# rasmusbarr/nudge

Measured on AMD Instinct MI355X. Metric: simulation steps/s (contacts solved/s alongside), 1M-box drop scene, higher is better.
Workload: dtype f32

## Files before the change

include/nudge_hip.h:

```cpp
#ifndef NUDGE_HIP_H
#define NUDGE_HIP_H

#include <stdint.h>

#ifdef __cplusplus
extern "C" {
#endif

enum {
	NH_OK = 0,
	NH_ERR_INVALID = 1,
	NH_ERR_NO_DEVICE = 2,
	NH_ERR_ARENA = 3,
	NH_ERR_CONTACT_CAPACITY = 4,
	NH_ERR_CACHE_CAPACITY = 5,
	NH_ERR_ACTIVE_CAPACITY = 6,
	NH_ERR_PAIR_CAPACITY = 7,
	NH_ERR_HIP = 8,
	NH_ERR_SCHEDULER_CAPACITY = 9,
	NH_ERR_STALE_HINT = 11,
	NH_ERR_STALE_SETUP = 10
};

enum {
// ... 50 lines not shown
typedef struct nh_ActiveBodies { uint32_t* indices; uint32_t capacity; uint32_t count; } nh_ActiveBodies;

typedef struct nh_ContactImpulseData nh_ContactImpulseData;
typedef struct nh_ContactConstraintData nh_ContactConstraintData;
typedef struct nh_context nh_context;

typedef struct nh_Counts {
	uint32_t colliders;
	uint32_t pairs;
	uint32_t contacts;
	uint32_t sleeping_pairs;
	uint32_t active_bodies;
	uint32_t cache;
	uint32_t culled;
	uint32_t large_colliders;
	uint32_t general_contacts;
	uint32_t levels;
	uint32_t error;
	uint32_t has_other_bodies;
	uint32_t unleveled;
	uint32_t raw_pairs;
	uint32_t broadphase_rebuilds;
	uint32_t sort_reuses;
	uint32_t broadphase_inserts;
	uint32_t still_steps;
	uint32_t still_replays;
	uint32_t still_diff[4];
	uint32_t blk_blocks, blk_bodies, blk_ghosts;
	uint32_t asleep_steps;
	uint32_t ahead_steps;
	uint32_t fused_steps;
	uint32_t pair_steps;
	uint32_t pair_diag[4];
} nh_Counts;

int nh_create(nh_context** out, int device, void* stream, uint32_t flags);
void nh_destroy(nh_context* ctx);
int nh_set_flags(nh_context* ctx, uint32_t flags);
int nh_synchronize(nh_context* ctx);
int nh_read_counts(nh_context* ctx, nh_Counts* out);
enum { NH_VIEW_CONTACTS = 1u , NH_VIEW_CACHE = 2u, NH_VIEW_ACTIVE = 4u , NH_VIEW_ALL = 7u };
int nh_export_views(nh_context* ctx, uint32_t what);
int nh_set_cache_count(nh_context* ctx, uint32_t count);
int nh_bodies_changed(nh_context* ctx);
int nh_set_tag_bits(nh_context* ctx, uint32_t bits);
int nh_set_pair_capacity(nh_context* ctx, uint32_t pairs);
int nh_set_option(nh_context* ctx, const char* name, int value);
const char* nh_error_string(int code);
int nh_last_hip_error(nh_context* ctx);

int nh_collide(nh_context* ctx, nh_ActiveBodies* active_bodies, nh_ContactData* contacts,
               const nh_BodyData* bodies, const nh_ColliderData* colliders,
               const nh_BodyConnections* body_connections, nh_Arena temporary);

int nh_append_contacts(nh_context* ctx, nh_ContactData* contacts, const nh_BodyData* bodies, uint32_t extra, uint32_t* positions, nh_Arena temporary);

int nh_apply_gravity_damping(nh_context* ctx, const nh_ActiveBodies* active_bodies, const nh_BodyData* bodies,
                             float time_step, const float gravity[3], float damping_rate);

int nh_read_cached_impulses(nh_context* ctx, const nh_ContactCache* contact_cache, const nh_ContactData* contacts,
                            nh_Arena* memory, nh_ContactImpulseData** out);

int nh_write_cached_impulses(nh_context* ctx, nh_ContactCache* contact_cache, const nh_ContactData* contacts,
                             nh_ContactImpulseData* contact_impulses);

int nh_setup_contact_constraints(nh_context* ctx, const nh_ActiveBodies* active_bodies, const nh_ContactData* contacts,
// ... 162 lines not shown
```

nudge_amd/csrc/nh_append.hip:

```cpp
#include "nh_internal.h"

__device__ __forceinline__ bool app_less(uint64_t ta, uint32_t fa, uint64_t tb, uint32_t fb) { return ta < tb || (ta == tb && fa < fb); }

__global__ __launch_bounds__(256) void k_app_rank(const nh_DevState* __restrict__ st, uint32_t extra, const uint64_t* __restrict__ tags, const uint32_t* __restrict__ features,
                                                  uint32_t* __restrict__ rank, uint64_t* __restrict__ skey, uint32_t* __restrict__ sfeat, uint32_t capacity) {
	const uint32_t K = st->contacts;
	if ((uint64_t)K + extra > capacity) return;
	for (uint32_t j = blockIdx.x * blockDim.x + threadIdx.x; j < extra; j += gridDim.x * blockDim.x) {
		const uint64_t t = tags[K + j]; const uint32_t f = features[K + j];
		uint32_t r = 0;
		for (uint32_t i = 0; i < extra; ++i) {
			const uint64_t ti = tags[K + i]; const uint32_t fi = features[K + i];
			r += (app_less(ti, fi, t, f) || (ti == t && fi == f && i < j)) ? 1u : 0u;
		}
		rank[j] = r; skey[r] = t; sfeat[r] = f;
	}
}

__global__ __launch_bounds__(256) void k_app_positions(const nh_DevState* __restrict__ st, uint32_t extra, const uint64_t* __restrict__ tags, const uint32_t* __restrict__ features,
                                                       const uint32_t* __restrict__ rank, const uint64_t* __restrict__ skey, const uint32_t* __restrict__ sfeat, uint32_t* __restrict__ pos, uint32_t capacity) {
	const uint32_t K = st->contacts;
	if ((uint64_t)K + extra > capacity) return;
	for (uint32_t i = blockIdx.x * blockDim.x + threadIdx.x; i < K + extra; i += gridDim.x * blockDim.x) {
		const uint64_t t = tags[i]; const uint32_t f = features[i];
// ... 26 lines not shown
	if ((uint64_t)st->contacts + extra > capacity) return;
	const uint32_t n = st->contacts + extra;
	for (uint32_t i = blockIdx.x * blockDim.x + threadIdx.x; i < n; i += gridDim.x * blockDim.x) {
		const uint32_t p = pos[i];
		reinterpret_cast<float4*>(data + p)[0] = t_data[2 * (size_t)i]; reinterpret_cast<float4*>(data + p)[1] = t_data[2 * (size_t)i + 1];
		bodies[p] = t_bodies[i]; tags[p] = t_tags[i]; features[p] = t_features[i];
	}
}

__global__ __launch_bounds__(256) void k_app_recount(nh_DevState* __restrict__ st, uint32_t extra, const nh_BodyPair* __restrict__ bodies, const uint64_t* __restrict__ tags,
                                                     uint32_t* __restrict__ deg, uint32_t nbodies, uint32_t capacity) {
	if ((uint64_t)st->contacts + extra > capacity) return;
	unsigned long long* __restrict__ pair_counter = reinterpret_cast<unsigned long long*>(deg + 2u * NH_DEG_STRIDE(nbodies));
	uint32_t* __restrict__ first_contact = deg + 4u * NH_DEG_STRIDE(nbodies);
	const uint32_t n = st->contacts + extra;
	for (uint32_t i = blockIdx.x * blockDim.x + threadIdx.x; i < n; i += gridDim.x * blockDim.x) {
		const nh_BodyPair p = bodies[i];
		if (i > 0 && tags[i - 1] == tags[i] && bodies[i - 1].a == p.a && bodies[i - 1].b == p.b) continue;
		const uint64_t t = tags[i];
		uint32_t len = 1;
		while (i + len < n && tags[i + len] == t && bodies[i + len].a == p.a && bodies[i + len].b == p.b) ++len;
		if (p.a) { atomicAdd(&pair_counter[p.a], (unsigned long long)len | ((unsigned long long)(p.b ? 0x10001u : 1u) << 32)); first_contact[p.a] = i | 0x80000000u; }
		if (p.b) { atomicAdd(&pair_counter[p.b], (unsigned long long)len | ((unsigned long long)(p.a ? 0x10001u : 1u) << 32)); first_contact[p.b] = i; }
	}
}

__global__ void k_app_count(nh_DevState* st, uint32_t extra, uint32_t capacity) {
	if (st->contacts + extra > capacity) st->error = NH_ERR_CONTACT_CAPACITY; else st->contacts += extra;
}

extern "C" int nh_append_contacts(nh_context* ctx, nh_ContactData* contacts, const nh_BodyData* bodies, uint32_t extra, uint32_t* positions, nh_Arena temporary) {
	if (!ctx || !contacts || !bodies) return NH_ERR_INVALID;
	if (!extra) return NH_OK;
	if (extra > 65536u || extra > contacts->capacity) return NH_ERR_INVALID;
	if (ctx->setup_seq == ctx->collide_seq || !ctx->deg) return NH_ERR_STALE_SETUP;
	{ int rc = nh_flush_pending(ctx); if (rc) return rc; }
	{ int rc = nh_still_sync_outputs(ctx); if (rc) return rc; }
	ctx->still.appended = true; ctx->still.ok_next = false;
	nh_DevState* st = ctx->d_state;
	const uint32_t cap = contacts->capacity, B = bodies->count;
	int err = NH_OK;
	uint32_t* rank = nh_arena_array<uint32_t>(&temporary, extra, &err);
	uint64_t* skey = nh_arena_array<uint64_t>(&temporary, extra, &err);
	uint32_t* sfeat = nh_arena_array<uint32_t>(&temporary, extra, &err);
	uint32_t* pos = positions ? positions : nh_arena_array<uint32_t>(&temporary, cap, &err);
	float4* t_data = nh_arena_array<float4>(&temporary, 2 * (size_t)cap, &err);
	nh_BodyPair* t_bodies = nh_arena_array<nh_BodyPair>(&temporary, cap, &err);
	uint64_t* t_tags = nh_arena_array<uint64_t>(&temporary, cap, &err);
	uint32_t* t_features = nh_arena_array<uint32_t>(&temporary, cap, &err);
	if (err) return err;
	if ((ctx->flags & NH_FLAG_SYNC_COUNTS) && (uint64_t)contacts->count + extra > cap) return NH_ERR_CONTACT_CAPACITY;
	NH_LAUNCH(ctx, "append_rank", k_app_rank, nh_grid_for(extra, 256, 1024), 256, st, extra, contacts->tags, contacts->features, rank, skey, sfeat, cap);
	NH_LAUNCH(ctx, "append_positions", k_app_positions, nh_grid_for(cap, 256, 2048), 256, st, extra, contacts->tags, contacts->features, rank, skey, sfeat, pos, cap);
	NH_LAUNCH(ctx, "append_copy", k_app_copy, nh_grid_for(cap, 256, 2048), 256, st, extra, contacts->data, contacts->bodies, contacts->tags, contacts->features, t_data, t_bodies, t_tags, t_features, cap);
	NH_LAUNCH(ctx, "append_scatter", k_app_scatter, nh_grid_for(cap, 256, 2048), 256, st, extra, pos, t_data, t_bodies, t_tags, t_features, contacts->data, contacts->bodies, contacts->tags, contacts->features, cap);
	NH_HIP_CHECK(ctx, hipMemsetAsync(ctx->deg, 0, sizeof(uint32_t) * NH_DEG_WORDS(B), ctx->stream));
	NH_LAUNCH(ctx, "append_recount", k_app_recount, nh_grid_for(cap, 256, 2048), 256, st, extra, contacts->bodies, contacts->tags, ctx->deg, B, cap);
	NH_LAUNCH(ctx, "append_count", k_app_count, 1, 1, st, extra, cap);
	if (ctx->flags & NH_FLAG_SYNC_COUNTS) {
		nh_Counts c;
		int rc = nh_read_counts(ctx, &c);
		if (rc) return rc;
		if (c.error) return (int)c.error;
		contacts->count = c.contacts;
	}
	return NH_OK;
// ... 2 lines not shown
```

nudge_amd/csrc/nh_cache.hip:

```cpp
#include "nh_internal.h"

__global__ __launch_bounds__(256) void k_cache_lookup(const nh_DevState* __restrict__ st, const uint64_t* __restrict__ tags, const uint32_t* __restrict__ features,
                                                      const uint64_t* __restrict__ ctags, const uint32_t* __restrict__ cfeatures, const nh_CachedContactImpulse* __restrict__ cdata,
                                                      nh_CachedContactImpulse* __restrict__ out, const nh_BodyPair* __restrict__ bodies, const uint8_t* __restrict__ body_class) {
	uint32_t n = st->contacts, m = st->cache;
	for (uint32_t i = blockIdx.x * blockDim.x + threadIdx.x; i < n; i += gridDim.x * blockDim.x) {
		if (body_class) {
			const nh_BodyPair p = bodies[i];
			const uint32_t ca = p.a ? body_class[p.a] : 0u, cb = p.b ? body_class[p.b] : 0u;
			if (ca != NH_CLS_GENERAL && cb != NH_CLS_GENERAL && ca != NH_CLS_STATICN && cb != NH_CLS_STATICN) continue;
		}
		uint64_t t = tags[i]; uint32_t f = features[i];
		uint32_t lo = 0, hi = m;
		if (i < m && ctags[i] == t && cfeatures[i] == f) { lo = i; hi = i; }
		while (lo < hi) { uint32_t mid = (lo + hi) >> 1; if (tag_less(ctags[mid], cfeatures[mid], t, f)) lo = mid + 1; else hi = mid; }
		nh_CachedContactImpulse r = { { 0.0f, 0.0f, 0.0f }, 0.0f };
		if (lo < m && ctags[lo] == t && cfeatures[lo] == f) r = cdata[lo];
		out[i] = r;
	}
}

__global__ __launch_bounds__(256) void k_cache_lookup_listed(const nh_DevState* __restrict__ st, const uint32_t* __restrict__ list, const uint64_t* __restrict__ tags, const uint32_t* __restrict__ features,
                                                             const uint64_t* __restrict__ ctags, const uint32_t* __restrict__ cfeatures, const nh_CachedContactImpulse* __restrict__ cdata,
                                                             nh_CachedContactImpulse* __restrict__ out) {
// ... 125 lines not shown
	}
}

__global__ __launch_bounds__(256) void k_sleep_undo(uint64_t* __restrict__ sc_undo, uint32_t* __restrict__ sc_count, uint32_t n, uint32_t confirmed_seq) {
	for (uint32_t r = blockIdx.x * blockDim.x + threadIdx.x; r < n; r += gridDim.x * blockDim.x) {
		const uint64_t u = sc_undo[r];
		if (u == 0ull) continue;
		if ((uint32_t)(u >> 32) > confirmed_seq) sc_count[r] = (uint32_t)u;
		sc_undo[r] = 0ull;
	}
}

static nh_ContactImpulseData* new_impulse_data(nh_context* ctx) {
	if (ctx->impulse_ring.empty()) { ctx->impulse_ring.resize(64, nullptr); ctx->constraint_ring.resize(64, nullptr); }
	uint32_t k = ctx->ring_pos % 64;
	if (!ctx->impulse_ring[k]) ctx->impulse_ring[k] = new nh_ContactImpulseData();
	return ctx->impulse_ring[k];
}

void nh_run_cull(nh_context* ctx, nh_ContactImpulseData* d, uint32_t sleeping_on_host) {
	if (!d->cull_pending) return;
	d->cull_pending = false;
	if (sleeping_on_host == 0) return;
	nh_DevState* st = ctx->d_state;
	const uint32_t ccap = d->cache_capacity;
	NH_LAUNCH(ctx, "cull_flags", k_cull_flags, nh_grid_for(ccap, 256, 4096), 256, st, d->ctags, d->sleeping_pairs, d->cull_flags);
	nh_scan_u32(ctx, d->cull_flags, d->cull_flags, &st->cache, 1, d->cull_tmp, &st->culled, &st->sleeping);
	NH_LAUNCH(ctx, "cull_write", k_cull_write, nh_grid_for(ccap, 256, 4096), 256, st, d->cull_flags, d->cull_flags, d->ctags, d->cfeatures, d->cdata,
	          d->culled_tags, d->culled_features, d->culled_data);
}

extern "C" int nh_read_cached_impulses(nh_context* ctx, const nh_ContactCache* cache, const nh_ContactData* contacts, nh_Arena* memory, nh_ContactImpulseData** out) {
	if (!ctx || !cache || !contacts || !memory || !out) return NH_ERR_INVALID;
	{
		const nh_StillStep& ss = ctx->still;
		const bool in_sequence = ss.active && !ss.resolved && !ctx->pending && cache->tags == ss.cache_tags && cache->features == ss.cache_features && cache->data == ss.cache_data &&
		                         cache->capacity == ss.cache_capacity && contacts->data == ss.lay_contacts.data && contacts->tags == ss.lay_contacts.tags;
		int rc = nh_flush_pending(ctx, true, in_sequence); if (rc) return rc;
	}
	const uint32_t kcap = contacts->capacity, ccap = cache->capacity;
	int err = NH_OK;
	ctx->ring_pos++;
	nh_ContactImpulseData* d = new_impulse_data(ctx);
	d->data = nh_arena_array<nh_CachedContactImpulse>(memory, kcap, &err);
	d->culled_tags = nh_arena_array<uint64_t>(memory, ccap, &err);
	d->culled_features = nh_arena_array<uint32_t>(memory, ccap, &err);
	d->culled_data = nh_arena_array<nh_CachedContactImpulse>(memory, ccap, &err);
	d->capacity = kcap; d->culled_capacity = ccap;
	d->cull_flags = nh_arena_array<uint32_t>(memory, ccap + 1, &err);
	d->cull_tmp = nh_arena_array<uint32_t>(memory, 2 * NH_SORT_GRID + 64, &err);
	if (err) return err;
	d->lookup_pending = true; d->ctx = ctx; d->consumed = false;
	d->tags = contacts->tags; d->features = contacts->features;
	d->ctags = cache->tags; d->cfeatures = cache->features; d->cdata = cache->data;
	d->cull_pending = contacts->sleeping_pairs != nullptr;
	d->sleeping_pairs = contacts->sleeping_pairs;
	d->cache_capacity = ccap;
	if (d->cull_pending && (ctx->flags & NH_FLAG_SYNC_COUNTS)) {
		nh_run_cull(ctx, d, ctx->h_state->sleeping);
	}
	*out = d;
	return NH_OK;
}

void nh_materialize_lookup(nh_context* ctx, nh_ContactImpulseData* d, const nh_BodyPair* bodies, const uint8_t* body_class, const uint32_t* general_list, uint32_t general) {
	if (!d->lookup_pending) return;
	d->lookup_pending = false;
	if (general_list && general != 0u && (uint64_t)general * 16u < d->capacity && !ctx->no_listed_lookup) {
		NH_LAUNCH(ctx, "cache_lookup_listed", k_cache_lookup_listed, nh_grid_for(general, 256, 4096), 256, ctx->d_state, general_list, d->tags, d->features, d->ctags, d->cfeatures, d->cdata, d->data);
		return;
	}
	NH_LAUNCH(ctx, "cache_lookup", k_cache_lookup, nh_grid_for(d->capacity, 256, 16384), 256, ctx->d_state, d->tags, d->features, d->ctags, d->cfeatures, d->cdata, d->data, bodies, body_class);
}

extern "C" const nh_CachedContactImpulse* nh_contact_impulses_device(const nh_ContactImpulseData* d) {
	if (!d) return nullptr;
	nh_ContactImpulseData* m = const_cast<nh_ContactImpulseData*>(d);
	if (m->ctx) {
		if (m->ctx->pending) nh_flush_pending(m->ctx);
		else if (!m->consumed) nh_materialize_lookup(m->ctx, m);
		nh_StillStep& ss = m->ctx->still;
		if (ss.active && ss.resolved && m->consumed && m->cdata == ss.cache_data) {
			if (nh_still_sync_outputs(m->ctx, NH_VIEW_CACHE) == NH_OK)
				hipMemcpyAsync(m->data, ss.cache.data, sizeof(nh_CachedContactImpulse) * (size_t)(m->capacity < ss.cache.capacity ? m->capacity : ss.cache.capacity), hipMemcpyDeviceToDevice, m->ctx->stream);
		}
	}
	return d->data;
}

extern "C" int nh_write_cached_impulses(nh_context* ctx, nh_ContactCache* cache, const nh_ContactData* contacts, nh_ContactImpulseData* imp) {
	if (!ctx || !cache || !contacts || !imp) return NH_ERR_INVALID;
	{ int rc = nh_flush_pending(ctx); if (rc) return rc; }
	{
		nh_StillStep& ss = ctx->still;
		if (ss.active && ss.resolved && cache->data == ss.cache_data && imp->ctx == ctx && imp->consumed) return NH_OK;
		ss.cache_ok = imp->consumed && !imp->cull_pending && !(ctx->flags & NH_FLAG_SYNC_COUNTS) && ((ctx->h_state->sleeping == 0u && ctx->h_state->culled == 0u) || !ss.no_local) &&
		              contacts->data == ss.lay_contacts.data && contacts->tags == ss.lay_contacts.tags;
		ss.cache_tags = cache->tags; ss.cache_features = cache->features; ss.cache_data = cache->data; ss.cache_capacity = cache->capacity;
		ss.cache = *cache;
		ss.slots_current = false;
	}
	if (!imp->consumed) nh_materialize_lookup(ctx, imp);
	if (imp->cull_pending) {
		nh_Counts c;
		int rc = nh_read_counts(ctx, &c);
		if (rc) return rc;
		nh_run_cull(ctx, imp, c.sleeping_pairs);
	}
	nh_DevState* st = ctx->d_state;
	NH_LAUNCH(ctx, "write_cache", k_write_cache, nh_grid_for((uint64_t)contacts->capacity + cache->capacity, 256, 4096), 256, st,
	          contacts->tags, contacts->features, imp->data, imp->culled_tags, imp->culled_features, imp->culled_data,
	          cache->tags, cache->features, cache->data, cache->capacity);
	if (ctx->still.ok_next && ctx->still.cache_ok && !ctx->still.disabled && (ctx->flags & NH_FLAG_FUSED_STEP) && ctx->sort_seeded) {
		NH_LAUNCH(ctx, "cache_to_slots", k_cache_to_slots, nh_grid_for(contacts->capacity, 256, 4096), 256, st, ctx->dense_slot, imp->data, contacts->features, ctx->rec,
		          ctx->sc_imp, ctx->sc_feat, ctx->sc_count);
		if (ctx->h_state->sleeping)
			NH_LAUNCH(ctx, "culled_to_slots", k_culled_to_slots, nh_grid_for(imp->culled_capacity, 256, 2048), 256, st, imp->culled_tags, imp->culled_features, imp->culled_data, ctx->sort_sorted_keys,
			          ctx->sort_sorted_idx, ctx->rec, ctx->lay_capacity, ctx->sc_imp, ctx->sc_feat, ctx->sc_count);
		ctx->still.slots_current = true;
	}
	if (ctx->flags & NH_FLAG_SYNC_COUNTS) {
		nh_Counts c;
		int rc = nh_read_counts(ctx, &c);
		if (rc) return rc;
// ... 28 lines not shown
```

nudge_amd/csrc/nh_collide.hip:

```cpp
#include "nh_internal.h"
#include "nh_narrowphase.h"
#include <type_traits>
#include "nh_solver.h"
#include <stdlib.h>

#define NH_ESC_MAX 4096u
#define NH_REINSERT_COMBOS(ncolliders) ((uint64_t)(ncolliders) * 16u)
#define NH_MOVED_MAX 16384u
__device__ __forceinline__ float nh_kept_margin(float cell_inv) { return cell_inv > 0.0f ? 0.03125f / cell_inv : 0.05f; }

template<bool STILL>
__global__ __launch_bounds__(1024) void k_xform(nh_DevState* __restrict__ st,
                                               const nh_Transform* __restrict__ body_xf,
                                               const nh_Transform* __restrict__ box_xf, const nh_BoxCollider* __restrict__ box_data, const uint32_t* __restrict__ box_tags, uint32_t nbox,
                                               const nh_Transform* __restrict__ sph_xf, const nh_SphereCollider* __restrict__ sph_data, const uint32_t* __restrict__ sph_tags, uint32_t nsph,
                                               nh_xform* __restrict__ xf, float4* __restrict__ aabb_min, float4* __restrict__ aabb_max, uint32_t* __restrict__ ctag,
                                               uint4* __restrict__ zero16, uint32_t zero16_count, float4* fat_box, uint32_t direct,
                                               uint8_t* __restrict__ gen, uint32_t* __restrict__ esc_mark, uint32_t* __restrict__ esc_list, uint32_t* __restrict__ moved_list, uint32_t seq,
                                               const uint8_t* __restrict__ idle = nullptr, uint32_t nbodies = 0u, uint32_t parity = 0u, uint8_t* __restrict__ awake_out = nullptr,
                                               uint32_t skip_asleep = 0u) {
	__shared__ uint32_t hist[STILL ? 1 : 1024];
	__shared__ uint32_t red[12];
	__shared__ uint32_t s_asleep;
	if (!STILL) hist[threadIdx.x] = 0;
// ... 1237 lines not shown
					for (int index = 0; index < 16; ++index) {
						if (((bb.mask >> index) & 1u) && k < count) {
							nh_contact_out o;
							nh_bb_contact(bb, index, bb.fx[index], bb.fy[index], bb.fz[index], bb.penetration[index], bb.tags[index], o);
							float4* dp = reinterpret_cast<float4*>(raw_data + base + k);
							dp[0] = make_float4(o.px, o.py, o.pz, o.penetration); dp[1] = make_float4(o.nx, o.ny, o.nz, o.friction);
							raw_feature[base + k] = o.feature;
							++k;
						}
					}
				} else {
					const nh_contact_out o = bb.kind == 1 ? bb.edge : single;
					float4* dp = reinterpret_cast<float4*>(raw_data + base);
					dp[0] = make_float4(o.px, o.py, o.pz, o.penetration); dp[1] = make_float4(o.nx, o.ny, o.nz, o.friction);
					raw_feature[base] = o.feature;
				}
			}
			rec[r].count = (uint32_t)count;
			if (old != (uint32_t)count) {
				cnt_sorted[pos] = (uint32_t)count;
				if (!st->delta_overflow[parity]) {
					const uint32_t k = atomicAdd(&st->delta_count[parity], 1u);
					if (k < NH_DELTA_MAX) delta[parity * NH_DELTA_MAX + k] = make_int2((int)pos, count - (int)old);
					else { st->delta_overflow[parity] = 1u; if (!delta_scan) changed = true; }
				}
			}
		}
		j += stride;
		if (j < n) r = list[j];
	}
	if (__ballot(changed) != 0ull && lane == 0) atomicMax(&st->still_failed_seq, seq);
}

__global__ __launch_bounds__(256) void k_asleep_check(nh_DevState* __restrict__ st, const nh_Transform* __restrict__ body_xf, const uint8_t* __restrict__ idle, uint32_t nbodies,
                                                      const nh_Transform* __restrict__ box_xf, const nh_BoxCollider* __restrict__ box_data, const uint32_t* __restrict__ box_tags, uint32_t nbox,
                                                      const nh_Transform* __restrict__ sph_xf, const nh_SphereCollider* __restrict__ sph_data, const uint32_t* __restrict__ sph_tags, uint32_t nsph,
                                                      const float4* __restrict__ was_min, const float4* __restrict__ was_max, const uint32_t* __restrict__ was_tag) {
	bool differs = false;
	for (uint32_t i = blockIdx.x * blockDim.x + threadIdx.x + 1u; i < nbodies; i += gridDim.x * blockDim.x) differs |= idle[i] != 0xffu;
	const uint32_t n = nbox + nsph;
	for (uint32_t c = blockIdx.x * blockDim.x + threadIdx.x; c < n; c += gridDim.x * blockDim.x) {
		const bool is_box = c < nbox;
		const nh_Transform l = is_box ? box_xf[c] : sph_xf[c - nbox];
		if (l.body >= nbodies) { differs = true; continue; }
		const nh_Transform b = body_xf[l.body];
		const nh_quat bq = { b.rotation[0], b.rotation[1], b.rotation[2], b.rotation[3] };
		const nh_quat lq = { l.rotation[0], l.rotation[1], l.rotation[2], l.rotation[3] };
		const nh_f3 p = nh_rotate(bq, nh_make3(l.position[0], l.position[1], l.position[2])) + nh_make3(b.position[0], b.position[1], b.position[2]);
		const nh_quat q = nh_qmul(bq, lq);
		float sx, sy, sz;
		uint32_t tag;
		if (is_box) {
			const nh_m33 m = nh_matrix(q);
			const nh_BoxCollider bc = box_data[c];
			const nh_f3 c0 = m.c0 * bc.size[0], c1 = m.c1 * bc.size[1], c2 = m.c2 * bc.size[2];
			sx = fabsf(c0.x) + fabsf(c1.x) + fabsf(c2.x);
			sy = fabsf(c0.y) + fabsf(c1.y) + fabsf(c2.y);
			sz = fabsf(c0.z) + fabsf(c1.z) + fabsf(c2.z);
			tag = box_tags[c];
		} else {
			sx = sy = sz = sph_data[c - nbox].radius;
			tag = sph_tags[c - nbox];
		}
		const float4 mn = was_min[c], mx = was_max[c];
		const float mnx = p.x - sx, mny = p.y - sy, mnz = p.z - sz, mxx = p.x + sx, mxy = p.y + sy, mxz = p.z + sz;
		differs |= __float_as_uint(mnx) != __float_as_uint(mn.x) || __float_as_uint(mny) != __float_as_uint(mn.y) || __float_as_uint(mnz) != __float_as_uint(mn.z) ||
// ... 279 lines not shown
	if (t == 0) {
		st->colliders = ncolliders; st->pairs = 0; st->pairs_sph = 0; st->raw_contacts = 0; st->records = 0; st->contacts = 0; st->sleeping = 0;
		st->active = 0; st->culled = 0; st->general_contacts = 0; st->levels = 0; st->error = 0;
		st->has_other = 0; st->has_unstable = 0; st->unleveled = 0; st->has_static8 = 0; st->has_staticN = 0; st->any_sleeping = 0; st->has_pending = 0;
		st->sort_buckets = st->sort_buckets_next;
		st->fat_escaped = 0; st->fat_rebuild = 0; st->esc_count = 0; st->fat_reinsert = 0;
		st->fat_hits_prev = st->fat_hits; st->fat_hits = 0;
		st->keys_changed = 0;
		if (drop_sort_order) st->sort_valid = 0;
		if (drop_kept_pairs) st->fat_valid = 0;
		for (int k = 0; k < 3; ++k) { st->smin[k] = 0xffffffffu; st->smax[k] = 0u; st->gmin[k] = 0xffffffffu; st->gmax[k] = 0u; }
	}
	for (uint32_t k = t; k < 1024u; k += blockDim.x) st->exp_hist[k] = 0;
}

static bool same_bodies(const nh_BodyData& a, const nh_BodyData& b) {
	return a.transforms == b.transforms && a.properties == b.properties && a.momentum == b.momentum && a.idle_counters == b.idle_counters && a.count == b.count;
}
static bool same_colliders(const nh_ColliderData& a, const nh_ColliderData& b) {
	return a.boxes.tags == b.boxes.tags && a.boxes.data == b.boxes.data && a.boxes.transforms == b.boxes.transforms && a.boxes.count == b.boxes.count &&
	       a.spheres.tags == b.spheres.tags && a.spheres.data == b.spheres.data && a.spheres.transforms == b.spheres.transforms && a.spheres.count == b.spheres.count;
}
static bool same_contacts(const nh_ContactData& a, const nh_ContactData& b) {
	return a.data == b.data && a.bodies == b.bodies && a.tags == b.tags && a.features == b.features && a.capacity == b.capacity && a.sleeping_pairs == b.sleeping_pairs;
}

static int collide_impl(nh_context* ctx, nh_ActiveBodies* active_bodies, nh_ContactData* contacts, const nh_BodyData* bodies, const nh_ColliderData* colliders,
                        const nh_BodyConnections* body_connections, nh_Arena temporary, bool want_still);

extern "C" int nh_collide(nh_context* ctx, nh_ActiveBodies* active_bodies, nh_ContactData* contacts,
                          const nh_BodyData* bodies, const nh_ColliderData* colliders,
                          const nh_BodyConnections* body_connections, nh_Arena temporary) {
	if (!ctx || !active_bodies || !contacts || !bodies || !colliders) return NH_ERR_INVALID;
	NH_HIP_CHECK(ctx, hipSetDevice(ctx->device));
	{ int rc = nh_flush_pending(ctx); if (rc) return rc; }
	nh_StillStep& ss = ctx->still;
	ss.active = false; ss.resolved = false; ss.setup_d = nullptr;
	const bool held = ss.hold != 0u;
	if (held) ss.hold--;
	const bool want_still = !held && !ss.disabled && !ctx->first_ghost && ss.ok_next && ss.cache_ok && ss.slots_current && !ss.appended && (ctx->flags & NH_FLAG_FUSED_STEP) && !(ctx->flags & (NH_FLAG_SYNC_COUNTS | NH_FLAG_EXACT_ORDER)) &&
	                        same_bodies(*bodies, ss.lay_bodies) && same_colliders(*colliders, ss.lay_colliders) && same_contacts(*contacts, ss.lay_contacts) &&
	                        active_bodies->indices == ss.lay_active && active_bodies->capacity == ss.lay_active_capacity;
	ss.active_out = active_bodies; ss.contacts_out = contacts; ss.bodies = *bodies; ss.colliders = *colliders;
	ss.has_connections = body_connections != nullptr;
	if (body_connections) ss.connections = *body_connections;
	ss.temporary = temporary;
	return collide_impl(ctx, active_bodies, contacts, bodies, colliders, body_connections, temporary, want_still);
}

int nh_still_collide_again(nh_context* ctx) {
	nh_StillStep& ss = ctx->still;
	const bool after_collide = ctx->after_collide, may_overlap = ctx->gravity_may_overlap;
	ss.active = false; ss.resolved = false; ss.ok_next = false;
	ss.failed++; ss.note_failure();
	ss.replaying = true;
	const int rc = collide_impl(ctx, ss.active_out, ss.contacts_out, &ss.bodies, &ss.colliders, ss.has_connections ? &ss.connections : nullptr, ss.temporary, false);
	ss.replaying = false;
	ctx->after_collide = after_collide; ctx->gravity_may_overlap = may_overlap;
	return rc;
}

int nh_still_view_contacts(nh_context* ctx) {
	const nh_ContactData& c = ctx->still.lay_contacts;
	const uint32_t pair_cap = ctx->lay_capacity;
	NH_LAUNCH(ctx, "gather_contacts", k_gather_contacts, nh_grid_for(pair_cap, 256, 8192), 256, ctx->d_state, ctx->sort_sorted_idx, ctx->rec, ctx->sort_sorted_keys, ctx->start_sorted,
	          ctx->raw_data, ctx->raw_feature, c.data, c.bodies, c.tags, c.features, c.capacity, pair_cap, (const uint32_t*)nullptr, (uint64_t*)nullptr, ctx->deg, ctx->still.bodies.count,
// ... 79 lines not shown
	return ctx->env_no_fat || ctx->bp_direct_left > 0;
}

static int reserve_kept(nh_context* ctx, const CollideCall& c, const CollideScratch& s, bool* fresh) {
	const uint32_t C = c.C, pair_cap = s.pair_cap;
	if (ctx->fat_nbox != c.nbox || ctx->fat_nsph != c.nsph) *fresh = true;
	const uint32_t want_kept = pair_cap > 0x7fffffffu / 2u ? 0xfffffffeu : (2u * pair_cap > 4096u ? 2u * pair_cap : 4096u);
	if (ctx->fat_pair_capacity != want_kept) {
		ctx->fat_pair_capacity = 0;
		{ int rc = nh_device_buffers(ctx, { { &ctx->fat_pairs, sizeof(uint2) * (size_t)want_kept } }); if (rc) return rc; }
		ctx->fat_pair_capacity = want_kept; *fresh = true;
	}
	if (ctx->fat_collider_capacity < C) {
		ctx->fat_collider_capacity = 0;
		{ int rc = nh_device_buffers(ctx, { { &ctx->fat_box, sizeof(float4) * 2u * (size_t)C } }); if (rc) return rc; }
		ctx->fat_collider_capacity = C; *fresh = true;
	}
	ctx->fat_nbox = c.nbox; ctx->fat_nsph = c.nsph;
	if (ctx->grid_cells < s.max_cells || ctx->grid_collider_capacity < ctx->fat_collider_capacity) {
		ctx->grid_cells = 0; ctx->grid_collider_capacity = 0;
		const size_t cc = ctx->fat_collider_capacity;
		const size_t cells = s.max_cells;
		{ int rc = nh_device_buffers(ctx, { { &ctx->grid_sbox, sizeof(float4) * 2u * cc + 64u }, { &ctx->grid_cstart, sizeof(uint32_t) * (cells + 8u) }, { &ctx->grid_counts, sizeof(uint32_t) * (cells + 8u), true },
		                                    { &ctx->grid_large, sizeof(uint32_t) * cc + 64u }, { &ctx->fat_gen, cc + 64u, true }, { &ctx->fat_esc_mark, sizeof(uint32_t) * cc + 64u, true },
		                                    { &ctx->fat_esc_list, sizeof(uint32_t) * NH_ESC_MAX }, { &ctx->fat_moved_list, sizeof(uint32_t) * NH_MOVED_MAX } }); if (rc) return rc; }
		ctx->grid_cells = s.max_cells; ctx->grid_collider_capacity = (uint32_t)cc; *fresh = true;
	}
	return NH_OK;
}

static int reserve_pair_layout(nh_context* ctx, uint32_t pair_cap, uint32_t cap, bool* fresh) {
	if (ctx->lay_capacity == pair_cap && ctx->lay_contact_capacity == cap) return NH_OK;
	ctx->lay_capacity = 0; ctx->lay_contact_capacity = 0;
	const size_t slots = (size_t)4 * pair_cap + cap, cache_slots = (size_t)5 * pair_cap + 64u, pairs = pair_cap;
	ctx->pair_list_capacity = pair_cap / 8u + 1024u;
	{ int rc = nh_device_buffers(ctx, { { &ctx->raw_data, sizeof(nh_Contact) * slots }, { &ctx->raw_feature, sizeof(uint32_t) * slots + 64u }, { &ctx->rec, sizeof(nh_Record) * pairs + 64u },
	                                    { &ctx->lay_rank, sizeof(uint32_t) * pairs + 64u }, { &ctx->cnt_sorted, sizeof(uint32_t) * (pairs + 2u) }, { &ctx->start_sorted, sizeof(uint32_t) * (pairs + 2u) },
	                                    { &ctx->dense_slot, sizeof(uint32_t) * (size_t)cap + 64u }, { &ctx->sc_imp, sizeof(float4) * cache_slots }, { &ctx->sc_feat, sizeof(uint32_t) * cache_slots },
	                                    { &ctx->sc_count, sizeof(uint32_t) * pairs + 64u }, { &ctx->sc_undo, sizeof(uint64_t) * pairs + 64u, true }, { &ctx->pair_mark, sizeof(uint32_t) * pairs + 64u, true },
	                                    { &ctx->pair_list, sizeof(uint32_t) * (size_t)ctx->pair_list_capacity }, { &ctx->exp_cnt, sizeof(uint32_t) * (pairs + 2u) }, { &ctx->exp_start, sizeof(uint32_t) * (pairs + 2u) },
	                                    { &ctx->exp_scan_tmp, sizeof(uint32_t) * (2u * NH_SORT_GRID + 64u) }, { &ctx->still_delta, sizeof(int2) * 2u * NH_DELTA_MAX } }); if (rc) return rc; }
	ctx->still.undo_dirty = false;
	ctx->raw_slots = (uint32_t)slots;
	ctx->lay_capacity = pair_cap; ctx->lay_contact_capacity = cap; *fresh = true;
	return NH_OK;
}

static int reserve_body_layout(nh_context* ctx, uint32_t B, bool* fresh) {
	if (ctx->lay_body_capacity >= B) return NH_OK;
	ctx->lay_body_capacity = 0;
	{ int rc = nh_device_buffers(ctx, { { &ctx->lay_class, (size_t)B + 64u }, { &ctx->lay_simple, sizeof(uint2) * (size_t)B + 64u }, { &ctx->body_rec, sizeof(uint32_t) * (size_t)B + 64u },
	                                    { &ctx->body_pos, sizeof(uint32_t) * (size_t)B + 64u } }); if (rc) return rc; }
	ctx->lay_body_capacity = B; *fresh = true;
	return NH_OK;
}

static int reserve_own(nh_context* ctx, uint32_t C) {
	if (ctx->own_capacity >= C) return NH_OK;
	ctx->own_capacity = 0;
	{ int rc = nh_device_buffers(ctx, { { &ctx->own_xf, sizeof(nh_xform) * (size_t)C + 64u }, { &ctx->own_aabb_min, sizeof(float4) * (size_t)C + 64u }, { &ctx->own_aabb_max, sizeof(float4) * (size_t)C + 64u },
	                                    { &ctx->own_ctag, sizeof(uint32_t) * (size_t)C + 64u } }); if (rc) return rc; }
	ctx->own_capacity = C; ctx->still.ahead_ready = false; ctx->still.own_current = false;
	return NH_OK;
}

struct StillForm {
	bool sleepers;
	bool movers;
	bool ahead_step;
	bool pair_step;
	bool take_map;
	bool list_unowned;
	bool early_verdict;
	bool delta_scan;
	bool local;
	uint32_t sleeper_skip;
};

static StillForm still_decide(nh_context* ctx, const CollideCall& c, const CollideMode& m) {
	nh_StillStep& ss = ctx->still;
	const uint32_t C = c.C, nbox = c.nbox, nsph = c.nsph;
	StillForm f;
	const bool sleepers = f.sleepers = !c.no_islands;
	ss.sleepers = sleepers;
	const bool movers = f.movers = m.incremental && !ss.no_local && ss.movers_left != 0u;
	if (ss.sleep_backoff) ss.sleep_backoff--;
	if (sleepers && !ss.was_sleepers) ss.sleep_stable = 0u;
	ss.was_sleepers = sleepers;
	const bool sleep_stable = sleepers && !ss.no_sleeper_ahead && !ss.no_pair && ss.sleep_stable >= 4u && ss.sleep_backoff == 0u && !ctx->step_hook && ss.pipelined && C <= (2u << 20);
	const bool plain = !movers && (!sleepers || sleep_stable) && !ss.appended_pairs && (nbox >= 2 || nsph != 0u);
	const bool ahead_step = f.ahead_step = plain && ss.ahead_ready && !ss.no_ahead && (!sleepers || ss.pair_ready);
	ss.ahead_ready = false; ss.ahead_plain = plain;
	const bool pair_step = f.pair_step = ahead_step && ss.pair_ready && !ss.no_pair;
	ss.pair_ready = false; ss.pair_step = pair_step; ss.early_verdict = false;
	if (pair_step) ss.pair_steps++;
	if (pair_step && sleepers && ss.sleep_run < 0xffffu) ss.sleep_run++;
	if (ahead_step) ss.ahead_steps++;
	f.sleeper_skip = (sleepers && ss.substep > 0u && ss.own_current && !ctx->step_hook && !ss.no_sleeper_skip) ? 1u : 0u;
	if (sleepers && !ahead_step) ss.ahead_map_ok = false;
	f.take_map = !ahead_step && plain && ss.more_steps && !ss.no_ahead && !ss.ahead_world_bad && !ss.ahead_map_ok && c.bodies->idle_counters;
	f.list_unowned = f.take_map && ss.pair_owned_seq == 0u && !ss.no_pair && ctx->pair_mark;
	f.delta_scan = C > (2u << 20) || (sleepers && !pair_step);
	if (sleepers) ss.undo_dirty = true;
	if (movers) ss.appended_pairs = true;
	f.local = sleepers || ss.appended_pairs;
	ss.own_current = sleepers;
	f.early_verdict = pair_step && ctx->step_hook && !ss.pipelined && ss.h_ring[0] && !ctx->timing;
	return f;
}

template<bool SPH, bool LOCAL>
static void launch_narrow_still(nh_context* ctx, const CollideCall& c, uint32_t pair_cap, const StillForm& f, const uint8_t* gen) {
	NH_LAUNCH(ctx, SPH ? "narrowphase_sph_still" : "narrowphase_still", (k_narrowphase<SPH, true, LOCAL>), nh_grid_for(pair_cap, 256, SPH ? 8192 : 4096), 256, ctx->d_state, ctx->fat_pairs, ctx->own_xf, ctx->own_ctag,
	          c.colliders->boxes.data, c.colliders->spheres.data, c.nbox, ctx->raw_data, ctx->raw_feature, pair_cap, 0u, ctx->sort_keys_by_position, ctx->rec, (uint32_t*)nullptr,
	          (const uint32_t*)nullptr, (const uint32_t*)nullptr, ctx->step_parity, 0u, ctx->fat_pair_capacity, ctx->own_aabb_min, ctx->own_aabb_max, gen, ctx->lay_rank, ctx->cnt_sorted, ctx->body_rec, ctx->collide_seq, ctx->still_delta, f.delta_scan ? 1u : 0u,
	           (LOCAL && f.sleepers) ? ctx->sc_count : (uint32_t*)nullptr,  (!LOCAL && f.ahead_step) ? 1u : 0u,  LOCAL ? ctx->sc_undo : (uint64_t*)nullptr,
	           LOCAL ? f.sleeper_skip : 0u);
}

static int still_launch(nh_context* ctx, const CollideCall& c, const CollideScratch& s, const CollideMode& m, const StillForm& f) {
	nh_StillStep& ss = ctx->still;
	nh_DevState* st = ctx->d_state;
	const nh_BodyData* bodies = c.bodies; const nh_ColliderData* colliders = c.colliders;
	const uint32_t C = c.C, B = c.B, nbox = c.nbox, nsph = c.nsph, pair_cap = s.pair_cap;
	nh_xform* xf = ctx->own_xf; float4* aabb_min = ctx->own_aabb_min; float4* aabb_max = ctx->own_aabb_max; uint32_t* ctag = ctx->own_ctag;
	if (!f.ahead_step)
		NH_LAUNCH(ctx, "xform_still", (k_xform<true>), nh_grid_for(C > B ? C : B, 1024, 256), 1024, st, bodies->transforms,
		          colliders->boxes.transforms, colliders->boxes.data, colliders->boxes.tags, nbox,
		          colliders->spheres.transforms, colliders->spheres.data, colliders->spheres.tags, nsph,
		          xf, aabb_min, aabb_max, ctag, (uint4*)nullptr, 0u, ctx->fat_box, 0u,
		          f.movers ? ctx->fat_gen : (uint8_t*)nullptr, ctx->fat_esc_mark, ctx->fat_esc_list, ctx->fat_moved_list, ctx->collide_seq, bodies->idle_counters, B, ctx->step_parity,
		          f.sleepers ? ctx->still_awake : (uint8_t*)nullptr, f.sleeper_skip);
	if (f.take_map) {
		{ int rc = reserve_one(ctx, &ctx->body_col, &ctx->body_col_capacity, B, sizeof(uint32_t) * (size_t)B + 64u); if (rc) return rc; }
		NH_HIP_CHECK(ctx, hipMemsetAsync(ctx->body_col, 0xff, sizeof(uint32_t) * (size_t)B, ctx->stream));
		NH_LAUNCH(ctx, "ahead_map", k_ahead_map, nh_grid_for(C, 256, 2048), 256, st, aabb_min, C, ctx->body_col);
		NH_LAUNCH(ctx, "ahead_check", k_ahead_check, nh_grid_for(C, 256, 1024), 256, st, aabb_min, C, ctx->body_col, f.sleepers ? bodies->idle_counters : (const uint8_t*)nullptr);
		if (f.list_unowned) {
			NH_HIP_CHECK(ctx, hipMemsetAsync(&st->pair_unowned, 0, sizeof(uint32_t), ctx->stream));
			NH_LAUNCH(ctx, "pair_mark", k_pair_mark, nh_grid_for(B, 256, 2048), 256, ctx->body_rec, (ctx->halo_ghost_first && ctx->halo_ghost_first < B) ? ctx->halo_ghost_first : B, ctx->pair_mark, ctx->collide_seq);
			NH_LAUNCH(ctx, "pair_list", k_pair_list, nh_grid_for(pair_cap, 256, 2048), 256, st, ctx->pair_mark, ctx->collide_seq, ctx->pair_list, ctx->pair_list_capacity, f.sleepers ? ctx->rec : (const nh_Record*)nullptr);
			ss.pair_owned_seq = ctx->collide_seq;
		}
		ss.ahead_map_ok = true;
	}
	if (f.movers)
		NH_LAUNCH(ctx, "reinsert_still", k_reinsert, 256, 256, st, nbox, ctx->grid_sbox, ctx->grid_cstart, ctx->grid_large, ctx->fat_box, ctx->fat_gen, ctx->fat_esc_mark, ctx->fat_esc_list,
		          ctx->fat_moved_list, ctx->collide_seq, ctx->fat_pairs, ctx->fat_pair_capacity, 1u, ctx->step_parity, C, ctx->body_rec, pair_cap);
	const uint8_t* gen = m.incremental ? ctx->fat_gen : (const uint8_t*)nullptr;
	if (f.pair_step) {
		const uint32_t pair_waves = ss.pair_world_ok ? std::min(std::max((ss.pair_listed + 63u) / 64u, 1u), 127u) : 127u;
		NH_LAUNCH(ctx, "pair_begin", k_pair_begin, 1u + pair_waves, 64, st, ctx->step_parity, ctx->collide_seq, ctx->pair_list, ctx->pair_list_capacity, ctx->fat_pairs, ctx->fat_pair_capacity, pair_cap, gen,
		          xf, aabb_min, aabb_max, ctag, colliders->boxes.data, colliders->spheres.data, nbox, ctx->sort_keys_by_position, ctx->rec,
		          ctx->lay_rank, ctx->cnt_sorted, ctx->body_rec, ctx->still_delta, ctx->raw_data, ctx->raw_feature, bodies->momentum, bodies->properties, f.delta_scan ? 1u : 0u, f.sleepers ? B : 0u);
		if (f.early_verdict) {
			NH_HIP_CHECK(ctx, hipMemcpyAsync(ss.h_ring[0], st, NH_COUNTER_WORDS * sizeof(uint32_t), hipMemcpyDeviceToHost, ctx->stream));
			NH_HIP_CHECK(ctx, hipEventRecord(ss.ev_ring[0], ctx->stream));
			ss.early_verdict = true;
		}
	} else {
		if (nbox >= 2) { if (f.local) launch_narrow_still<false, true>(ctx, c, pair_cap, f, gen); else launch_narrow_still<false, false>(ctx, c, pair_cap, f, gen); }
		if (nsph) { if (f.local) launch_narrow_still<true, true>(ctx, c, pair_cap, f, gen); else launch_narrow_still<true, false>(ctx, c, pair_cap, f, gen); }
	}
	if (f.delta_scan) nh_scan_u32(ctx, ctx->cnt_sorted, ctx->start_sorted, &st->records, 1, s.scan_tmp, nullptr, &st->delta_overflow[ctx->step_parity]);
	return NH_OK;
}

static void full_find_contacts(nh_context* ctx, const CollideCall& c, const CollideScratch& s, const CollideMode& m, bool seeded_sort) {
	nh_DevState* st = ctx->d_state;
	const nh_BodyData* bodies = c.bodies; const nh_ColliderData* colliders = c.colliders; const nh_BodyConnections* body_connections = c.body_connections;
	const uint32_t C = c.C, B = c.B, nbox = c.nbox, nsph = c.nsph, pair_cap = s.pair_cap, max_cells = s.max_cells;
	const bool bp_direct = m.bp_direct, incremental = m.incremental, no_islands = c.no_islands;
	NH_LAUNCH(ctx, "xform_aabb", (k_xform<false>), nh_grid_for(C, 1024, 256), 1024, st, bodies->transforms,
	          colliders->boxes.transforms, colliders->boxes.data, colliders->boxes.tags, nbox,
	          colliders->spheres.transforms, colliders->spheres.data, colliders->spheres.tags, nsph,
	          s.xf, s.aabb_min, s.aabb_max, s.ctag, (uint4*)nullptr, 0u, ctx->fat_box, bp_direct ? 1u : 0u,
	          incremental ? ctx->fat_gen : (uint8_t*)nullptr, ctx->fat_esc_mark, ctx->fat_esc_list, ctx->fat_moved_list, ctx->collide_seq);
	if (ctx->asleep.streak >= 1u && !ctx->asleep.disabled) (void)asleep_snapshot(ctx);
	NH_LAUNCH(ctx, "grid_setup", k_grid_setup, 1, 64, st, C, max_cells, bp_direct ? 1u : 0u, ctx->fat_pair_capacity);
	float4* fbox = ctx->fat_box;
	float4* sbox = ctx->grid_sbox; uint32_t* large_list = ctx->grid_large; uint32_t* cell_start = ctx->grid_cstart; uint32_t* cstart = ctx->grid_counts;
	uint2* kept = ctx->fat_pairs;
// ... 104 lines not shown
		if (n.error) return (int)n.error;
	}
	ctx->gravity_may_overlap = ctx->side != nullptr;
	ctx->after_collide = true;
	return NH_OK;
}

static int collide_impl(nh_context* ctx, nh_ActiveBodies* active_bodies, nh_ContactData* contacts, const nh_BodyData* bodies, const nh_ColliderData* colliders,
                        const nh_BodyConnections* body_connections, nh_Arena temporary, bool want_still) {
	ctx->adv.done = false;
	ctx->step_parity ^= 1u;
	ctx->collide_seq++;
	ctx->collide_mark = ctx->advance_count;
	CollideCall c = { active_bodies, contacts, bodies, colliders, body_connections };
	c.no_islands = ctx->idle_bound >= 0 && (uint64_t)ctx->idle_bound + (ctx->advance_count - ctx->idle_bound_mark) < 0xffu;
	ctx->islands_skipped = c.no_islands;
	ctx->idle_unknown = false;
	c.nbox = colliders->boxes.count; c.nsph = colliders->spheres.count; c.C = c.nbox + c.nsph; c.B = bodies->count; c.cap = contacts->capacity;
	ctx->body_count = c.B;
	CollideScratch s;
	{ int rc = carve_scratch(ctx, c, temporary, &s); if (rc) return rc; }
	CollideMode m = {};
	m.drop_sort_order = ctx->env_no_sort_reuse;
	{ int rc = reserve_one(ctx, &ctx->deg, &ctx->deg_capacity, (uint32_t)NH_DEG_WORDS(c.B), sizeof(uint32_t) * NH_DEG_WORDS(c.B)); if (rc) return rc; }
	{ int rc = reserve_sort(ctx, s.pair_cap, &m.drop_sort_order); if (rc) return rc; }
	m.bp_direct = broadphase_direct(ctx);
	{ int rc = reserve_kept(ctx, c, s, &m.drop_kept); if (rc) return rc; }
	m.incremental = !m.bp_direct && !ctx->env_no_incremental && c.C < (1u << NH_GEN_SHIFT);
	bool lay_fresh = false;
	{ int rc = reserve_pair_layout(ctx, s.pair_cap, c.cap, &lay_fresh); if (rc) return rc; }
	{ int rc = reserve_body_layout(ctx, c.B, &lay_fresh); if (rc) return rc; }
	nh_StillStep& ss = ctx->still;
	if (lay_fresh) { ss.slots_current = false; ss.ok_next = false; }
	if (!same_colliders(*colliders, ss.lay_colliders)) ss.ahead_world_bad = false;
	ss.lay_bodies = *bodies; ss.lay_colliders = *colliders; ss.lay_contacts = *contacts; ss.lay_active = active_bodies->indices; ss.lay_active_capacity = active_bodies->capacity;
	ss.appended = false;
	const bool may_sleep = !c.no_islands;
	const bool sleepers_ok = !ss.no_local && !(body_connections && body_connections->count);
	if (may_sleep && sleepers_ok) { int rc = reserve_one(ctx, &ctx->still_awake, &ctx->still_awake_capacity, c.B, (size_t)c.B + 64u); if (rc) return rc; }
	const bool still = want_still && (c.no_islands || sleepers_ok) && !m.bp_direct && !m.drop_kept && !m.drop_sort_order && !lay_fresh && ctx->sort_seeded && !ctx->env_sort_radix &&
	                   !ctx->env_no_sort_reuse && c.C != 0u;
	if (!still) return full_step(ctx, c, s, m);
	{ int rc = reserve_own(ctx, c.C); if (rc) return rc; }
	const StillForm f = still_decide(ctx, c, m);
	{ int rc = still_launch(ctx, c, s, m, f); if (rc) return rc; }
	ss.active = true; ss.resolved = false; ss.launched++;
	ctx->gravity_may_overlap = false;
	ctx->after_collide = true;
	return NH_OK;
}
```

nudge_amd/csrc/nh_context.hip:

```cpp
#include "nh_internal.h"
#include <stdlib.h>
#include <string.h>

extern "C" int nh_create(nh_context** out, int device, void* stream, uint32_t flags) {
	if (!out) return NH_ERR_INVALID;
	int count = 0;
	if (hipGetDeviceCount(&count) != hipSuccess || count <= 0 || device < 0 || device >= count) return NH_ERR_NO_DEVICE;
	if (hipSetDevice(device) != hipSuccess) return NH_ERR_NO_DEVICE;
	nh_context* ctx = new nh_context();
	ctx->device = device;
	ctx->stream = (hipStream_t)stream;
	ctx->asleep.streak = 0;
	ctx->flags = (flags & NH_FLAG_FUSED_STEP) ? (flags | NH_FLAG_SINGLE_APPLY) : flags;
	ctx->after_collide = false; ctx->grav.pending = false; ctx->grav.rest_pending = false; ctx->adv.done = false; ctx->adv.rest = true;
	ctx->tag_bits = 32;
	ctx->last_hip_error = 0;
	ctx->timing = false;
	ctx->timing_current = false;
	ctx->ring_pos = 0;
	ctx->body_count = 0;
	ctx->pending = nullptr;
	ctx->hint = nullptr;
	ctx->hint_capacity = 0;
	ctx->deg = nullptr;
	ctx->deg_capacity = 0;
	ctx->order_seq = 0;
	ctx->sort_splitters = nullptr; ctx->sort_counts = nullptr; ctx->sort_starts = nullptr; ctx->sort_capacity = 0; ctx->sort_seeded = false;
	ctx->step_parity = 0;
	ctx->pair_capacity = 0;
	ctx->collide_seq = 0; ctx->setup_seq = 0;
	ctx->idle_bound = -1; ctx->idle_unknown = true; ctx->advance_count = 0; ctx->collide_mark = 0; ctx->idle_bound_mark = 0; ctx->islands_skipped = false;
	ctx->sort_tile = 0u; ctx->sort_target = 0u;
	ctx->env_sort_radix = false;
	ctx->env_no_sort_reuse = false;
	ctx->sort_keys_by_position = nullptr; ctx->sort_sorted_keys = nullptr; ctx->sort_sorted_idx = nullptr;
	ctx->bp_seen_rebuilds = 0; ctx->bp_rebuild_streak = 0; ctx->bp_direct_left = 0;
	ctx->env_no_fat = false;
	ctx->fat_pairs = nullptr; ctx->fat_pair_capacity = 0; ctx->fat_box = nullptr; ctx->fat_collider_capacity = 0; ctx->fat_nbox = ctx->fat_nsph = 0xffffffffu;
	ctx->grid_sbox = nullptr; ctx->grid_skeys = nullptr; ctx->grid_cstart = nullptr; ctx->grid_counts = nullptr; ctx->grid_large = nullptr; ctx->grid_cells = 0; ctx->grid_collider_capacity = 0;
	ctx->fat_gen = nullptr; ctx->fat_esc_mark = nullptr; ctx->fat_esc_list = nullptr; ctx->fat_moved_list = nullptr;
	ctx->env_blk_rows_global = false; ctx->sync_exports_views = false;
	ctx->env_blk_global_colours = false; ctx->last_general_contacts = 0;
	ctx->env_no_incremental = false;
	ctx->env_colour_check_seeds = false;
	ctx->env_no_resident = false;
	ctx->os_resident = 0;
	memset(&ctx->blk, 0, sizeof(ctx->blk));
	ctx->blk.scale = 1.0f;
	ctx->blk.disabled = false; ctx->blk.check = false;
	ctx->blk.chain = true;
	ctx->blk.min_contacts = 200000u;
	ctx->blk.target = 900u;
	ctx->raw_data = nullptr; ctx->raw_feature = nullptr; ctx->raw_slots = 0; ctx->rec = nullptr; ctx->lay_rank = nullptr; ctx->cnt_sorted = nullptr; ctx->start_sorted = nullptr; ctx->dense_slot = nullptr;
	ctx->sc_imp = nullptr; ctx->sc_feat = nullptr; ctx->sc_count = nullptr; ctx->sc_undo = nullptr; ctx->pair_mark = nullptr; ctx->pair_list = nullptr; ctx->pair_list_capacity = 0; ctx->exp_cnt = nullptr; ctx->exp_start = nullptr; ctx->exp_scan_tmp = nullptr; ctx->still_delta = nullptr; ctx->lay_capacity = 0; ctx->lay_contact_capacity = 0;
	ctx->own_xf = nullptr; ctx->own_aabb_min = nullptr; ctx->own_aabb_max = nullptr; ctx->own_ctag = nullptr; ctx->own_capacity = 0; ctx->body_col = nullptr; ctx->body_col_capacity = 0;
	ctx->still_awake = nullptr; ctx->still_awake_capacity = 0; ctx->exp_sleep_a = nullptr; ctx->exp_sleep_b = nullptr; ctx->exp_sleep_hist = nullptr; ctx->exp_flags = nullptr; ctx->exp_sleep_capacity = 0; ctx->exp_flags_capacity = 0;
	ctx->lay_class = nullptr; ctx->lay_simple = nullptr; ctx->body_rec = nullptr; ctx->body_pos = nullptr; ctx->lay_body_capacity = 0;
	memset(&ctx->still, 0, sizeof(ctx->still));
	ctx->step_hook = nullptr; ctx->step_hook_user = nullptr; ctx->halo_ghost_first = 0u;
	ctx->first_ghost = 0;
	memset(&ctx->asleep, 0, sizeof(ctx->asleep));
	memset(&ctx->stream_state, 0, sizeof(ctx->stream_state)); ctx->stream_state.last_slot = -1;
	{ int cus = 0; ctx->cu_count = (hipDeviceGetAttribute(&cus, hipDeviceAttributeMultiprocessorCount, ctx->device) == hipSuccess && cus > 0) ? cus : 256; }
	ctx->d_state = nullptr;
	ctx->h_state = nullptr;
	if (hipMalloc((void**)&ctx->d_state, sizeof(nh_DevState)) != hipSuccess) { delete ctx; return NH_ERR_HIP; }
	if (hipHostMalloc((void**)&ctx->h_state, sizeof(nh_DevState), 0) != hipSuccess) { hipFree(ctx->d_state); delete ctx; return NH_ERR_HIP; }
	memset(ctx->h_state, 0, sizeof(nh_DevState));
	ctx->h_early = nullptr; ctx->no_early_counts = false; ctx->early_reads = 0; ctx->early_fallbacks = 0;
	if (hipHostMalloc((void**)&ctx->h_early, sizeof(uint32_t) * (NH_COUNTER_WORDS + 16u), 0) != hipSuccess) { ctx->h_early = nullptr; (void)hipGetLastError(); }
	else memset(ctx->h_early, 0, sizeof(uint32_t) * (NH_COUNTER_WORDS + 16u));
	ctx->side = nullptr; ctx->ev_fork = nullptr; ctx->ev_join = nullptr; ctx->ev_active = nullptr; ctx->ev_gravity = nullptr; ctx->gravity_may_overlap = false;
	if (hipStreamCreateWithFlags(&ctx->side, hipStreamNonBlocking) != hipSuccess || hipEventCreateWithFlags(&ctx->ev_fork, hipEventDisableTiming) != hipSuccess ||
	    hipEventCreateWithFlags(&ctx->ev_join, hipEventDisableTiming) != hipSuccess || hipEventCreateWithFlags(&ctx->ev_active, hipEventDisableTiming) != hipSuccess ||
	    hipEventCreateWithFlags(&ctx->ev_gravity, hipEventDisableTiming) != hipSuccess) { ctx->side = nullptr; }
	hipMemsetAsync(ctx->d_state, 0, sizeof(nh_DevState), ctx->stream);
	hipStreamSynchronize(ctx->stream);
	*out = ctx;
	return NH_OK;
}

extern "C" void nh_destroy(nh_context* ctx) {
	if (!ctx) return;
	hipSetDevice(ctx->device);
	hipStreamSynchronize(ctx->stream);
	for (auto& s : ctx->timer_slots) { ctx->event_pool.push_back(s.a); ctx->event_pool.push_back(s.b); }
	for (auto e : ctx->event_pool) hipEventDestroy(e);
	for (auto p : ctx->impulse_ring) delete p;
	for (auto p : ctx->constraint_ring) delete p;
	if (ctx->side) { hipStreamSynchronize(ctx->side); hipStreamDestroy(ctx->side); }
	if (ctx->ev_fork) hipEventDestroy(ctx->ev_fork);
	if (ctx->ev_join) hipEventDestroy(ctx->ev_join);
	if (ctx->ev_active) hipEventDestroy(ctx->ev_active);
	if (ctx->ev_gravity) hipEventDestroy(ctx->ev_gravity);
	{
		nh_StateStream& ss = ctx->stream_state;
		if (ss.stage) hipFree(ss.stage);
		if (ss.staged) hipEventDestroy(ss.staged);
		for (int k = 0; k < NH_STREAM_MAX_SLOTS; ++k) if (ss.landed[k]) hipEventDestroy(ss.landed[k]);
	}
	for (int k = 0; k < 2; ++k) { if (ctx->still.h_ring[k]) hipHostFree(ctx->still.h_ring[k]); if (ctx->still.ev_ring[k]) hipEventDestroy(ctx->still.ev_ring[k]); }
	nh_query_free(ctx);
	{
		void* bufs[] = { ctx->asleep.aabb_min, ctx->asleep.aabb_max, ctx->asleep.tags, ctx->hint, ctx->deg, ctx->fat_pairs, ctx->fat_box, ctx->grid_sbox, ctx->grid_skeys, ctx->grid_cstart, ctx->grid_counts, ctx->grid_large, ctx->fat_gen,
		                 ctx->fat_esc_mark, ctx->fat_esc_list, ctx->fat_moved_list, ctx->sort_keys_by_position, ctx->sort_sorted_keys, ctx->sort_sorted_idx, ctx->sort_splitters, ctx->sort_counts, ctx->sort_starts,
		                 ctx->raw_data, ctx->raw_feature, ctx->rec, ctx->lay_rank, ctx->cnt_sorted, ctx->start_sorted, ctx->dense_slot, ctx->sc_imp, ctx->sc_feat, ctx->sc_count, ctx->sc_undo, ctx->pair_mark, ctx->pair_list, ctx->exp_cnt, ctx->exp_start,
		                 ctx->exp_scan_tmp, ctx->still_delta, ctx->lay_class, ctx->lay_simple, ctx->body_rec, ctx->body_pos, ctx->still_awake, ctx->exp_sleep_a, ctx->exp_sleep_b, ctx->exp_sleep_hist, ctx->exp_flags,
		                 ctx->own_xf, ctx->own_aabb_min, ctx->own_aabb_max, ctx->own_ctag, ctx->body_col };
		for (void* b : bufs) if (b) hipFree(b);
	}
	{
		nh_BlkBuffers& k = ctx->blk;
		void* bufs[] = { k.brank, k.bm, k.pos_body, k.touch, k.lpair, k.ghost_list, k.blk_count, k.own_base, k.bins, k.bin_off, k.ghost_base, k.ghost_count, k.phase_list, k.desc, k.scan_tmp, k.prof, k.chain_slot, k.chain_nbr, k.chain_done, k.chain_ticket };
		for (void* b : bufs) if (b) hipFree(b);
	}
	if (ctx->d_state) hipFree(ctx->d_state);
	if (ctx->h_state) hipHostFree(ctx->h_state);
	if (ctx->h_early) hipHostFree(ctx->h_early);
	delete ctx;
}

extern "C" int nh_set_flags(nh_context* ctx, uint32_t flags) {
	if (!ctx) return NH_ERR_INVALID;
	{ int rc = nh_flush_pending(ctx); if (rc) return rc; }
	ctx->asleep.streak = 0;
	ctx->flags = (flags & NH_FLAG_FUSED_STEP) ? (flags | NH_FLAG_SINGLE_APPLY) : flags;
	return NH_OK;
}
extern "C" int nh_set_first_ghost_body(nh_context* ctx, uint32_t first_ghost) {
	if (!ctx) return NH_ERR_INVALID;
	{ int rc = nh_flush_pending(ctx); if (rc) return rc; }
	ctx->asleep.streak = 0;
	ctx->first_ghost = first_ghost;
	return NH_OK;
}

extern "C" int nh_set_option(nh_context* ctx, const char* name, int value) {
	if (!ctx || !name) return NH_ERR_INVALID;
	{ int rc = nh_flush_pending(ctx); if (rc) return rc; }
	const std::string n(name);
	const bool on = value != 0;
	ctx->asleep.streak = 0;
	if (n == "no_asleep") ctx->asleep.disabled = on;
	else if (n == "sync_exports_views") ctx->sync_exports_views = on;
	else if (n == "no_early_counts") ctx->no_early_counts = on;
	else if (n == "no_listed_lookup") ctx->no_listed_lookup = on;
	else if (n == "no_sleeper_ahead") ctx->still.no_sleeper_ahead = on;
	else if (n == "no_sleeper_skip") ctx->still.no_sleeper_skip = on;
	else if (n == "halo_overlap") ctx->halo_overlap = on;
	else if (n == "no_pair_ahead") ctx->still.no_pair = on;
	else if (n == "no_xform_ahead") ctx->still.no_ahead = on;
	else if (n == "no_local_still") ctx->still.no_local = on;
	else if (n == "no_still") ctx->still.disabled = on;
	else if (n == "sort_radix") ctx->env_sort_radix = on;
	else if (n == "no_sort_reuse") ctx->env_no_sort_reuse = on;
	else if (n == "bucket_tile") ctx->sort_tile = (uint32_t)value;
	else if (n == "bucket_target") ctx->sort_target = (uint32_t)value;
	else if (n == "colour_check_seeds") ctx->env_colour_check_seeds = on;
	else if (n == "no_kept_pairs") ctx->env_no_fat = on;
	else if (n == "no_incremental") ctx->env_no_incremental = on;
	else if (n == "no_resident") ctx->env_no_resident = on;
	else if (n == "no_blocks") ctx->blk.disabled = on;
	else if (n == "blk_check") ctx->blk.check = on;
	else if (n == "blk_min") ctx->blk.min_contacts = (uint32_t)value;
	else if (n == "blk_target") ctx->blk.target = value < 8 ? 8u : (uint32_t)value;
	else if (n == "blk_rows_global") ctx->env_blk_rows_global = on;
	else if (n == "blk_global_colours") ctx->env_blk_global_colours = on;
	else if (n == "no_blk_chain") ctx->blk.chain = !on;
	else if (n == "blk_profile") {
		if (on && !ctx->blk.prof) NH_HIP_CHECK(ctx, hipMalloc((void**)&ctx->blk.prof, sizeof(unsigned long long) * 4u * 8u * NH_BLK_MAX_BLOCKS));
	}
	else return NH_ERR_INVALID;
	return NH_OK;
}

extern "C" int nh_set_tag_bits(nh_context* ctx, uint32_t bits) { if (!ctx || bits < 1 || bits > 32) return NH_ERR_INVALID; ctx->tag_bits = bits; return NH_OK; }

extern "C" int nh_bodies_changed(nh_context* ctx) {
	if (!ctx) return NH_ERR_INVALID;
	{ int rc = nh_still_abandon(ctx); if (rc) return rc; }
	ctx->idle_bound = -1; ctx->idle_unknown = true;
	ctx->asleep.streak = 0;
	ctx->still.ok_next = false;
	ctx->still.own_current = false;
	ctx->still.sleep_backoff = 0u; ctx->still.sleep_stable = 0u;
	return NH_OK;
}

extern "C" int nh_set_pair_capacity(nh_context* ctx, uint32_t pairs) { if (!ctx) return NH_ERR_INVALID; ctx->pair_capacity = pairs; return NH_OK; }

extern "C" int nh_synchronize(nh_context* ctx) {
	if (!ctx) return NH_ERR_INVALID;
	int rc = nh_flush_pending(ctx);
	if (rc) return rc;
	if (ctx->sync_exports_views) { rc = nh_still_sync_outputs(ctx, NH_VIEW_ALL); if (rc) return rc; }
	NH_HIP_CHECK(ctx, hipStreamSynchronize(ctx->stream));
	if (ctx->timing) nh_timer_collect(ctx);
	return NH_OK;
}

void nh_counts_from_mirror(nh_context* ctx, nh_Counts* out) {
	const nh_DevState* h = ctx->h_state;
	if (ctx->collide_seq && !ctx->idle_unknown) { ctx->idle_bound = (int)h->max_idle[ctx->step_parity]; ctx->idle_bound_mark = ctx->collide_mark; }
	out->colliders = h->colliders; out->pairs = h->pairs + h->pairs_sph; out->contacts = h->contacts; out->sleeping_pairs = h->sleeping;
	out->active_bodies = h->active; out->cache = h->cache; out->culled = h->culled; out->large_colliders = h->large;
	if (ctx->still.cache_stale) out->cache = h->contacts + h->culled;
	out->general_contacts = h->general_contacts; out->levels = h->levels; out->error = h->error;
	out->still_steps = (uint32_t)(ctx->still.launched - ctx->still.failed - ((ctx->still.active && !ctx->still.resolved) ? 1u : 0u)); out->still_replays = (uint32_t)ctx->still.failed;
	for (int k = 0; k < 4; ++k) out->still_diff[k] = h->still_diff[k];
	out->asleep_steps = (uint32_t)ctx->asleep.steps; out->ahead_steps = (uint32_t)ctx->still.ahead_steps; out->fused_steps = 0u; out->pair_steps = (uint32_t)ctx->still.pair_steps;
	for (int k = 0; k < 4; ++k) out->pair_diag[k] = h->pair_diag[k];
	out->blk_blocks = h->blk.nblk; out->blk_bodies = h->blk.bodies; out->blk_ghosts = h->blk.ghost_cursor;
	out->has_other_bodies = h->has_other; out->broadphase_rebuilds = h->fat_rebuilds; out->sort_reuses = h->sort_reuses; out->broadphase_inserts = h->fat_inserts; out->unleveled = h->unleveled; out->raw_pairs = h->pairs + h->pairs_sph;
}

extern "C" int nh_read_counts(nh_context* ctx, nh_Counts* out) {
	if (!ctx || !out) return NH_ERR_INVALID;
	{ int rc = nh_flush_pending(ctx, true); if (rc) return rc; }
	if (ctx->sync_exports_views) { int rc = nh_still_sync_outputs(ctx, NH_VIEW_ALL); if (rc) return rc; }
	NH_HIP_CHECK(ctx, hipMemcpyAsync(ctx->h_state, ctx->d_state, NH_COUNTER_WORDS * sizeof(uint32_t), hipMemcpyDeviceToHost, ctx->stream));
	NH_HIP_CHECK(ctx, hipStreamSynchronize(ctx->stream));
	nh_counts_from_mirror(ctx, out);
	if (ctx->timing) nh_timer_collect(ctx);
	return NH_OK;
}

__global__ void k_set_cache_count(nh_DevState* st, uint32_t n) { st->cache = n; }

extern "C" int nh_set_cache_count(nh_context* ctx, uint32_t count) {
	if (!ctx) return NH_ERR_INVALID;
	{ int rc = nh_still_abandon(ctx); if (rc) return rc; }
	ctx->asleep.streak = 0;
	ctx->still.cache_ok = false; ctx->still.slots_current = false; ctx->still.cache_stale = false;
	hipLaunchKernelGGL(k_set_cache_count, dim3(1), dim3(1), 0, ctx->stream, ctx->d_state, count);
	return NH_OK;
}

extern "C" int nh_stream_state(nh_context* ctx, const nh_BodyData* bodies, uint32_t count, void* host_ring, uint32_t slots, uint32_t every) {
	if (!ctx) return NH_ERR_INVALID;
	NH_HIP_CHECK(ctx, hipSetDevice(ctx->device));
	nh_StateStream& ss = ctx->stream_state;
	if (ctx->side) NH_HIP_CHECK(ctx, hipStreamSynchronize(ctx->side));
	for (int k = 0; k < NH_STREAM_MAX_SLOTS; ++k) { ss.in_flight[k] = false; ss.slot_frame[k] = 0; ss.slot_step[k] = 0; }
	ss.every = 0; ss.last_slot = -1; ss.advances = 0; ss.frames = 0; ss.dropped = 0;
	if (every == 0u) return NH_OK;
	if (!bodies || !bodies->transforms || !host_ring || count == 0u || count > bodies->count || slots == 0u || slots > NH_STREAM_MAX_SLOTS || !ctx->side) return NH_ERR_INVALID;
	if (ss.stage_capacity < count) {
		ss.stage_capacity = 0;
		{ int rc = nh_device_buffers(ctx, { { &ss.stage, sizeof(nh_Transform) * (size_t)count } }); if (rc) return rc; }
		ss.stage_capacity = count;
	}
	if (!ss.staged) NH_HIP_CHECK(ctx, hipEventCreateWithFlags(&ss.staged, hipEventDisableTiming));
	for (uint32_t k = 0; k < slots; ++k) if (!ss.landed[k]) NH_HIP_CHECK(ctx, hipEventCreateWithFlags(&ss.landed[k], hipEventDisableTiming));
	ss.src = bodies->transforms; ss.count = count; ss.ring = static_cast<char*>(host_ring); ss.slots = slots; ss.every = every;
	return NH_OK;
}

int nh_stream_after_advance(nh_context* ctx) {
	nh_StateStream& ss = ctx->stream_state;
	if (!ss.every) return NH_OK;
	ss.advances++;
	if (ss.advances % ss.every) return NH_OK;
	const uint32_t slot = (uint32_t)(ss.frames % ss.slots);
	const int prev = ss.last_slot;
// ... 58 lines not shown

void nh_timer_begin(nh_context* ctx, const char* name) {
	ctx->timing_current = ctx->timing_filter.empty() || ctx->timing_filter == name;
	if (!ctx->timing_current) return;
	nh_TimerSlot s;
	s.name = name;
	s.a = take_event(ctx);
	s.b = take_event(ctx);
	hipEventRecord(s.a, ctx->stream);
	ctx->timer_slots.push_back(s);
}

void nh_timer_end(nh_context* ctx) {
	if (!ctx->timing_current) return;
	hipEventRecord(ctx->timer_slots.back().b, ctx->stream);
}

void nh_timer_collect(nh_context* ctx) {
	for (auto& s : ctx->timer_slots) {
		float ms = 0.0f;
		if (hipEventElapsedTime(&ms, s.a, s.b) == hipSuccess) {
			auto& acc = ctx->kernel_ms[s.name];
			acc.first += ms;
			acc.second += 1;
		}
		ctx->event_pool.push_back(s.a);
		ctx->event_pool.push_back(s.b);
	}
	ctx->timer_slots.clear();
}

extern "C" int nh_enable_timing(nh_context* ctx, int on) {
	if (!ctx) return NH_ERR_INVALID;
	hipStreamSynchronize(ctx->stream);
	if (ctx->timing) nh_timer_collect(ctx);
	ctx->timing = on != 0;
	return NH_OK;
}

extern "C" int nh_set_timing_filter(nh_context* ctx, const char* name) {
	if (!ctx) return NH_ERR_INVALID;
	ctx->timing_filter = name ? name : "";
	return NH_OK;
}

extern "C" int nh_kernel_times(nh_context* ctx, nh_KernelTime* out, int cap, int reset) {
	if (!ctx) return 0;
	hipStreamSynchronize(ctx->stream);
	nh_timer_collect(ctx);
	int n = 0;
	ctx->name_store.clear();
	ctx->name_store.reserve(ctx->kernel_ms.size());
	for (auto& kv : ctx->kernel_ms) {
		if (n >= cap) break;
		ctx->name_store.push_back(kv.first);
		out[n].name = ctx->name_store.back().c_str();
		out[n].ms = kv.second.first;
		out[n].launches = kv.second.second;
		out[n].reserved = 0;
		++n;
	}
	if (reset) ctx->kernel_ms.clear();
	return n;
}
```

nudge_amd/csrc/nh_internal.h:

```cpp
#ifndef NH_INTERNAL_H
#define NH_INTERNAL_H

#include <hip/hip_runtime.h>
#include <stdint.h>
#include <stdio.h>
#include <string>
#include <vector>
#include <map>

#include "../../include/nudge_hip.h"
#include "nh_math.h"

#define NH_WAVE 64
#define NH_BLOCK 256
#define NH_MAX_CELLS 0xFFFFFFu
#define NH_LARGE_KEY 0xFFFFFFu
#define NH_SORT_GRID 512
#define NH_MAX_LEVELS 4096

#define NH_BLK_ID_BITS 15u
#define NH_BLK_MAX_BLOCKS (1u << NH_BLK_ID_BITS)
#define NH_BLK_MAX_COLOURS 32u
#define NH_BLK_RADIAL 0x8000u
struct nh_BlkGrid {
// ... 61 lines not shown
	uint32_t records_kept, records_prev;
	uint32_t sort_valid;
	uint32_t smin[3];
	uint32_t smax[3];
	uint32_t gmin[3];
	uint32_t gmax[3];
	float morton_scale;
	float morton_min[3];
	float cell_inv;
	float origin[3];
	uint32_t dims[3];
	uint32_t small_exp;
	uint32_t redo_small;
	uint32_t exp_hist[1024];
	uint32_t any_idle[2];
	uint32_t sort_buckets;
	uint32_t sort_buckets_next;
	uint32_t colour_cursor;
	uint32_t stale_hint;
	uint32_t order_conflict;
	uint32_t lay_in_place;
	uint32_t delta_count[2], delta_overflow[2];
	uint32_t still_smin[2][3], still_smax[2][3];
	uint32_t asleep_failed;
	uint32_t still_top[2];
	uint32_t still_esc[2];
	uint32_t still_fat0;
	uint32_t still_asleep[2], still_sleeping[2], still_culled[2];
	uint32_t sleep_part[2][64][2];
	uint32_t ahead_failed_seq;
	uint32_t still_static_min[3], still_static_max[3];
	uint32_t ahead_part[2][64][8];
	nh_BlkGrid blk;
};

struct nh_TimerSlot { const char* name; hipEvent_t a, b; };

#define NH_AHEAD_PARTS 64u
#define NH_SLEEP_PARTS 64u
struct nh_xform;
struct nh_AheadView { const uint32_t* body_col; const nh_Transform* box_xf; const nh_BoxCollider* box_data; const nh_Transform* sph_xf; const nh_SphereCollider* sph_data; uint32_t nbox;
                      nh_xform* xf; float4* aabb_min; float4* aabb_max; const float4* fat_box;
                      const uint2* kept; uint32_t kept_cap, pair_cap; const uint64_t* rec_key; const uint32_t* ctag; const uint8_t* gen;
                      struct nh_Record* rec; nh_Contact* raw_data; uint32_t* raw_feature; uint32_t* cnt_sorted; int2* delta; uint32_t unowned_cap, delta_scan; };
struct nh_FusedStep { float gx_dt, gy_dt, gz_dt, damping, time_step; uint32_t bits; uint8_t* idle; uint32_t seq, guard_seq;
                      uint32_t ghost_first;
                      uint32_t* host_counters;
                      uint32_t part; const uint32_t* xlist; const uint32_t* xcount; const uint8_t* xskip; };

struct nh_BlkBuffers {
	uint2* brank;
	float4* bm;
	uint32_t* pos_body;
	uint32_t* touch;
	uint32_t body_capacity;
	uint32_t* lpair;
	uint32_t* ghost_list;
	uint32_t contact_capacity;
	uint32_t* blk_count; uint32_t* own_base;
	uint32_t* bins; uint32_t* bin_off;
	uint32_t* ghost_base; uint32_t* ghost_count;
	uint32_t* phase_list;
	uint32_t* desc;
	uint32_t* scan_tmp;
	bool tables;
	float scale;
// ... 25 lines not shown
	bool early_verdict;
	bool pair_ready;
	bool pair_step;
	bool no_pair;
	uint32_t pair_owned_seq;
	bool pair_world_bad;
	bool pair_world_ok;
	uint32_t pair_listed;
	uint64_t pair_steps;
	uint32_t steps_left;
	uint32_t confirmed_seq;
	bool undo_dirty;
	uint32_t hold, fail_level, good_run;
	uint32_t seen_inserts, seen_rebuilds;
	bool no_local; uint32_t movers_left;
	bool no_ahead;
	bool more_steps;
	bool ahead_map_ok;
	bool ahead_world_bad;
	bool ahead_plain;
	bool ahead_ready;
	uint64_t ahead_steps;
	bool appended_pairs;
	bool sleepers;
	uint32_t substep;
	bool no_sleeper_ahead;
	bool was_sleepers;
	uint32_t sleep_backoff_len, sleep_run;
	uint32_t sleep_last_active, sleep_stable, sleep_backoff;
	bool no_sleeper_skip;
	bool own_current;
	bool views_sleepers;
	bool sleep_pairs_current, active_current;
	void note_failure() { hold = (1u << fail_level) - 1u; if (fail_level < 6u) ++fail_level; good_run = 0; }
	void note_confirmed() { if (++good_run >= 16u) fail_level = 0; }
};

struct nh_AsleepState {
	bool disabled;
	uint32_t streak;
	uint32_t prev_pairs, prev_sleeping, prev_cache;
	float4 *aabb_min, *aabb_max; uint32_t* tags; uint32_t capacity;
	uint32_t C, B;
	uint32_t snap_C, snap_seq;
	const float4 *last_aabb_min, *last_aabb_max; const uint32_t* last_ctag; uint32_t last_C;
	uint64_t steps;
};

#define NH_STREAM_MAX_SLOTS 16
struct nh_StateStream {
	uint32_t every, slots, count; const nh_Transform* src; char* ring;
	nh_Transform* stage; uint32_t stage_capacity;
	hipEvent_t staged, landed[NH_STREAM_MAX_SLOTS]; bool in_flight[NH_STREAM_MAX_SLOTS];
	uint64_t slot_step[NH_STREAM_MAX_SLOTS], slot_frame[NH_STREAM_MAX_SLOTS];
	uint64_t advances, frames, dropped; int last_slot;
};

struct nh_context {
	int device;
	int cu_count;
	hipStream_t stream;
	uint32_t flags;
	uint32_t tag_bits;
	nh_DevState* d_state;
	nh_DevState* h_state;
	uint32_t* h_early;
// ... 40 lines not shown
	uint64_t advance_count, collide_mark, idle_bound_mark;
	bool islands_skipped;
	bool env_sort_radix, env_no_resident, env_colour_check_seeds;
	int os_resident;
	uint64_t* sort_splitters;
	uint32_t* sort_counts;
	uint32_t* sort_starts;
	uint32_t sort_capacity;
	uint32_t sort_tile, sort_target;
	bool sort_seeded;
	hipStream_t side;
	hipEvent_t ev_fork, ev_join;
	hipEvent_t ev_active, ev_gravity;
	bool gravity_may_overlap;
	bool after_collide;
	struct { bool pending, rest_pending; float gx_dt, gy_dt, gz_dt, damping, time_step; const uint32_t* active; nh_BodyMomentum* momentum; uint32_t body_count; } grav;
	struct { bool done, rest; float time_step; const uint8_t* body_class; } adv;
	nh_BlkBuffers blk;
	nh_Contact* raw_data; uint32_t* raw_feature; uint32_t raw_slots;
	struct nh_Record* rec;
	uint32_t* lay_rank;
	uint32_t* cnt_sorted; uint32_t* start_sorted;
	uint32_t* dense_slot;
	float4* sc_imp; uint32_t* sc_feat; uint32_t* sc_count;
	uint64_t* sc_undo;
	struct nh_xform* own_xf; float4* own_aabb_min; float4* own_aabb_max; uint32_t* own_ctag; uint32_t own_capacity;
	uint32_t* body_col; uint32_t body_col_capacity;
	uint32_t* pair_mark; uint32_t* pair_list; uint32_t pair_list_capacity;
	uint8_t* still_awake; uint32_t still_awake_capacity;
	uint64_t* exp_sleep_a; uint64_t* exp_sleep_b; uint32_t* exp_sleep_hist; uint32_t* exp_flags; uint32_t exp_sleep_capacity, exp_flags_capacity;
	int2* still_delta;
	uint32_t* exp_cnt; uint32_t* exp_start; uint32_t* exp_scan_tmp;
	uint32_t lay_capacity, lay_contact_capacity;
	uint8_t* lay_class; uint2* lay_simple; uint32_t* body_rec; uint32_t* body_pos; uint32_t lay_body_capacity;
	nh_StillStep still;
	int (*step_hook)(nh_context* ctx, void* user, uint32_t sub_step); void* step_hook_user; uint32_t halo_ghost_first;
	struct { bool armed, launched; hipStream_t stream; const uint32_t* list; const uint32_t* count; const uint8_t* mask; uint32_t bound;
	         int (*after_verdict)(nh_context* ctx, void* user); void* user; } halo_split;
	bool halo_overlap;
	nh_AsleepState asleep;
	uint32_t first_ghost;
	nh_StateStream stream_state;
	struct nh_QueryState* query;
};
int nh_stream_after_advance(nh_context* ctx);
void nh_query_free(nh_context* ctx);

#define NH_LOCAL __attribute__((visibility("hidden")))
int nh_flush_pending(nh_context* ctx, bool keep_gravity = false, bool in_sequence = false);
int nh_still_abandon(nh_context* ctx);
int nh_still_sync_outputs(nh_context* ctx, uint32_t what = 7u );
int nh_still_export_cache(nh_context* ctx);
int nh_still_undo_drops(nh_context* ctx);
void nh_stream_void_advance(nh_context* ctx);
int nh_still_verdict_now(nh_context* ctx);
int nh_still_await_number(nh_context* ctx);
NH_LOCAL void nh_still_note_movers(nh_context* ctx, const nh_DevState* h, uint32_t seq = 0u);
int nh_asleep_remember(nh_context* ctx);
int nh_asleep_verify(nh_context* ctx, const nh_BodyData* bodies, const nh_ColliderData* colliders);
int nh_still_collide_again(nh_context* ctx);
int nh_still_view_contacts(nh_context* ctx);
struct nh_ContactImpulseData;
NH_LOCAL void nh_run_cull(nh_context* ctx, nh_ContactImpulseData* d, uint32_t sleeping_on_host);
NH_LOCAL void nh_materialize_lookup(nh_context* ctx, nh_ContactImpulseData* d, const nh_BodyPair* bodies = nullptr, const uint8_t* body_class = nullptr, const uint32_t* general_list = nullptr, uint32_t general = 0u);
#define NH_INTERNAL_STILL_FAILED (-1000)
#define NH_DELTA_MAX 256u
#define NH_GEN_SHIFT 24u
#define NH_GEN_INDEX 0xFFFFFFu
#define NH_BODY_REC_NONE 0xFFFFFFFFu
#define NH_BODY_REC_IS_A 0x80000000u
struct nh_Record { uint32_t body_a, body_b, overflow, count; };
#define NH_REC_SLEEPING 0x80000000u
void nh_counts_from_mirror(nh_context* ctx, nh_Counts* out);
#define NH_COUNTER_WORDS 41u

struct nh_ContactImpulseData {
	nh_CachedContactImpulse* data;
	bool lookup_pending;
	bool consumed;
	nh_context* ctx;
	const uint64_t* tags; const uint32_t* features;
	const uint64_t* ctags; const uint32_t* cfeatures; const nh_CachedContactImpulse* cdata;
	uint64_t* culled_tags;
	uint32_t* culled_features;
	nh_CachedContactImpulse* culled_data;
	uint32_t capacity;
	bool cull_pending;
	const uint64_t* sleeping_pairs;
	uint32_t* cull_flags; uint32_t* cull_tmp;
	uint32_t cache_capacity;
	uint32_t culled_capacity;
};

struct nh_ContactConstraintData {
// ... 181 lines not shown
```

nudge_amd/csrc/nh_partition.hip:

```cpp
#include "nh_internal.h"
#include "nh_math.h"
#include <math.h>
#include <string.h>

struct nh_PartDev {
	uint32_t zero;
	uint32_t count[2];
	uint32_t kinds[2];
	uint32_t vmax_bits;
	float kth[2];
	uint32_t error;
};

struct nh_PartCollider { float shape[4]; nh_Transform cxf; uint32_t tag; uint32_t pad; };
struct nh_FullRecord { nh_Transform xf; nh_BodyProperties props; nh_BodyMomentum momentum; nh_PartCollider col[NH_PARTITION_MAX_COLLIDERS]; uint8_t nbox, nsph, idle, pad; };
static_assert(sizeof(nh_PartCollider) == 56 && sizeof(nh_FullRecord) == NH_PARTITION_FULL_BYTES, "full record layout");
#define NP_MAXC NH_PARTITION_MAX_COLLIDERS

struct nh_partition {
	nh_context* ctx;
	nh_PartitionConfig cfg;
	double lo, hi, cut0[2];
	uint32_t n_owned, n_bodies, n_boxes, n_spheres;
	uint32_t ghost_out[2], ghost_in[2];
// ... 932 lines not shown
		o[2] = make_float4(m0.y, m0.z, m0.w, m1.x);
		o[3] = make_float4(m1.y, m1.z, m1.w, __uint_as_float((uint32_t)idle[i]));
	}
}

__global__ __launch_bounds__(256) void k_halo_unpack(nh_Transform* __restrict__ xf, nh_BodyMomentum* __restrict__ momentum, uint8_t* __restrict__ idle,
                                                     uint32_t first_slot, uint32_t count, const nh_HaloRecord* __restrict__ in) {
	for (uint32_t k = blockIdx.x * blockDim.x + threadIdx.x; k < count; k += gridDim.x * blockDim.x) {
		const uint32_t i = first_slot + k;
		const float4* r = reinterpret_cast<const float4*>(in + k);
		const float4 a = r[0], b = r[1], c = r[2], d = r[3];
		nh_Transform* t = xf + i;
		t->position[0] = a.x; t->position[1] = a.y; t->position[2] = a.z;
		reinterpret_cast<float4*>(t)[1] = make_float4(a.w, b.x, b.y, b.z);
		reinterpret_cast<float4*>(momentum + i)[0] = make_float4(b.w, c.x, c.y, c.z);
		reinterpret_cast<float4*>(momentum + i)[1] = make_float4(c.w, d.x, d.y, d.z);
		idle[i] = (uint8_t)__float_as_uint(d.w);
	}
}

extern "C" int nh_halo_pack(nh_context* ctx, const nh_BodyData* bodies, const uint32_t* indices, uint32_t count, void* out) {
	if (!ctx || !bodies || (count && (!indices || !out))) return NH_ERR_INVALID;
	{ int rc = nh_flush_pending(ctx); if (rc) return rc; }
	if (count) NH_LAUNCH(ctx, "halo_pack", k_halo_pack, nh_grid_for(count, 256, 1024), 256, bodies->transforms, bodies->momentum, bodies->idle_counters, indices, count, (nh_HaloRecord*)out);
	return NH_OK;
}

static int halo_unpack(nh_context* ctx, const nh_BodyData* bodies, uint32_t first_slot, uint32_t count, const void* in, bool same_bodies);
extern "C" int nh_halo_update(nh_context* ctx, const nh_BodyData* bodies, uint32_t first_slot, uint32_t count, const void* in) { return halo_unpack(ctx, bodies, first_slot, count, in, true); }
extern "C" int nh_halo_unpack(nh_context* ctx, const nh_BodyData* bodies, uint32_t first_slot, uint32_t count, const void* in) { return halo_unpack(ctx, bodies, first_slot, count, in, false); }

static int halo_unpack(nh_context* ctx, const nh_BodyData* bodies, uint32_t first_slot, uint32_t count, const void* in, bool same_bodies) {
	if (!ctx || !bodies || (count && !in) || (uint64_t)first_slot + count > bodies->count) return NH_ERR_INVALID;
	{ int rc = nh_flush_pending(ctx); if (rc) return rc; }
	if (count && !same_bodies) { ctx->idle_bound = -1; ctx->idle_unknown = true; }
	if (count) NH_LAUNCH(ctx, "halo_unpack", k_halo_unpack, nh_grid_for(count, 256, 1024), 256, bodies->transforms, bodies->momentum, bodies->idle_counters, first_slot, count, (const nh_HaloRecord*)in);
	return NH_OK;
}

void nh_halo_pack_on(hipStream_t stream, const nh_BodyData* bodies, const uint32_t* indices, uint32_t count, void* out) {
	if (count) hipLaunchKernelGGL(k_halo_pack, dim3(nh_grid_for(count, 256, 1024)), dim3(256), 0, stream, bodies->transforms, bodies->momentum, bodies->idle_counters, indices, count, (nh_HaloRecord*)out);
}
void nh_halo_update_on(hipStream_t stream, const nh_BodyData* bodies, uint32_t first_slot, uint32_t count, const void* in) {
	if (count) hipLaunchKernelGGL(k_halo_unpack, dim3(nh_grid_for(count, 256, 1024)), dim3(256), 0, stream, bodies->transforms, bodies->momentum, bodies->idle_counters, first_slot, count, (const nh_HaloRecord*)in);
}
```

nudge_amd/csrc/nh_schedule.hip:

```cpp
#include "nh_internal.h"
#include "nh_solver.h"

#define NH_FIRST_IS_A 0x80000000u
__global__ __launch_bounds__(256) void k_adj_simple(nh_DevState* __restrict__ st, uint32_t nbodies, uint32_t* __restrict__ deg, const unsigned long long* __restrict__ pair_counter,
                                                    const uint32_t* __restrict__ first_contact, const uint32_t* __restrict__ slot_key,
                                                    uint8_t* __restrict__ body_class, const nh_BodyProperties* __restrict__ props, nh_BodyMomentum* __restrict__ momentum,
                                                    uint2* __restrict__ simple, uint32_t* __restrict__ body_rec, uint32_t* __restrict__ body_pos, const uint32_t* __restrict__ sorted_idx) {
	bool other = false, unstable = false;
	for (uint32_t x = blockIdx.x * blockDim.x + threadIdx.x; x < nbodies; x += gridDim.x * blockDim.x) {
		if (x == 0) {
			body_class[0] = 0;
			momentum[0].unused0 = props[0].mass_inverse;
			const nh_BodyMomentum m0 = momentum[0];
			const nh_BodyProperties p0 = props[0];
			st->static_inert = nh_is_inert(m0.velocity, m0.angular_velocity, p0.inertia_inverse, p0.mass_inverse) ? 1u : 0u;
			deg[0] = 0u;
			continue;
		}
		const unsigned long long pc = pair_counter[x];
		const uint32_t d = (uint32_t)pc;
		deg[x] = d;
		uint32_t cls = NH_CLS_NONE;
		if (d) {
			const uint32_t inf = (uint32_t)(pc >> 32);
// ... 154 lines not shown
			if (lane == 0) emitted = e + 1;
			changed = true;
		}
		__syncthreads();
		if (changed) {
			if (lane == 0) vacancy[bucket] = vac;
			if (lane < 8) S.set_ab(bucket, vac, lane, make_uint2(NH_NONE, NH_NONE));
		}
		__syncthreads();
	}
	uint32_t e = emitted;
	for (uint32_t b = 0; b < GR_BUCKETS; ++b) {
		uint32_t vac = vacancy[b];
		for (uint32_t j = 0; j < vac; ++j) {
			if (lane < 8) {
				uint2 ab = S.ab(b, j, lane);
				if (!(ab.x == NH_NONE && ab.y == NH_NONE)) slot_key[S.idx(b, j, lane)] = e;
			}
			++e;
		}
	}
}

static nh_ContactConstraintData* new_constraint_data(nh_context* ctx) {
	if (ctx->constraint_ring.empty()) { ctx->impulse_ring.resize(64, nullptr); ctx->constraint_ring.resize(64, nullptr); }
	uint32_t k = ctx->ring_pos % 64;
	if (!ctx->constraint_ring[k]) ctx->constraint_ring[k] = new nh_ContactConstraintData();
	return ctx->constraint_ring[k];
}

extern "C" int nh_setup_contact_constraints(nh_context* ctx, const nh_ActiveBodies* active_bodies, const nh_ContactData* contacts,
                                            const nh_BodyData* bodies, nh_ContactImpulseData* imp, nh_Arena* memory, nh_ContactConstraintData** out) {
	if (!ctx || !contacts || !bodies || !imp || !memory || !out) return NH_ERR_INVALID;
	{
		const nh_StillStep& ss = ctx->still;
		const bool in_sequence = ss.active && !ss.resolved && !ctx->pending && contacts->data == ss.lay_contacts.data && contacts->bodies == ss.lay_contacts.bodies &&
		                         bodies->momentum == ss.bodies.momentum && bodies->transforms == ss.bodies.transforms && bodies->count == ss.bodies.count && imp->ctx == ctx && !imp->consumed;
		int rc = nh_flush_pending(ctx, true, in_sequence); if (rc) return rc;
	}
	(void)active_bodies;
	nh_DevState* st = ctx->d_state;
	const uint32_t kcap = contacts->capacity;
	const uint32_t B = bodies->count;
	int err = NH_OK;
	nh_ContactConstraintData* d = new_constraint_data(ctx);
	d->rows = nh_arena_array<float>(memory, (size_t)kcap * 40, &err);
	d->states = nh_arena_array<float>(memory, (size_t)kcap * 4, &err);
	if (!ctx->deg || ctx->deg_capacity < NH_DEG_WORDS(B)) return NH_ERR_INVALID;
	if (ctx->setup_seq == ctx->collide_seq) return NH_ERR_STALE_SETUP;
	if ((ctx->flags & NH_FLAG_SYNC_COUNTS) && contacts->count != ctx->h_state->contacts) return NH_ERR_STALE_SETUP;
	ctx->setup_seq = ctx->collide_seq;
	d->body_off = nh_arena_array<uint32_t>(memory, (size_t)B + 2u, &err);
	d->adj = nh_arena_array<uint32_t>(memory, (size_t)kcap * 2, &err);
	if (!ctx->lay_class || ctx->lay_body_capacity < B) return NH_ERR_INVALID;
	d->body_class = ctx->lay_class;
	d->simple = ctx->lay_simple;
	d->level_order = nh_arena_array<uint32_t>(memory, kcap, &err);
	d->gpair = nh_arena_array<uint2>(memory, kcap, &err);
	d->gstates = nh_arena_array<float4>(memory, kcap, &err);
	uint32_t* cursor = ctx->deg + NH_DEG_STRIDE(B);
	uint32_t* pred_a = nh_arena_array<uint32_t>(memory, kcap, &err);
	uint32_t* pred_b = nh_arena_array<uint32_t>(memory, kcap, &err);
	uint32_t* level = nh_arena_array<uint32_t>(memory, kcap, &err);
	uint32_t* general_list = nh_arena_array<uint32_t>(memory, kcap, &err);
	uint32_t* slot_key = (ctx->flags & NH_FLAG_EXACT_ORDER) ? nh_arena_array<uint32_t>(memory, kcap, &err) : nullptr;
	uint32_t* tent = (ctx->flags & NH_FLAG_EXACT_ORDER) ? nullptr : nh_arena_array<uint32_t>(memory, kcap, &err);
// ... 12 lines not shown
	d->csr_ready = false;
	if (slot_key) {
		const uint32_t seq = ++ctx->order_seq ? ctx->order_seq : ++ctx->order_seq;
		NH_LAUNCH(ctx, "order_check", k_order_check, nh_grid_for(kcap / 8u + 16u, 256, 1024), 256, st, contacts->bodies, slot_key, seq);
		NH_LAUNCH(ctx, "greedy_replay", k_greedy_replay, 1, 64, st, contacts->bodies, slot_key, seq, spill_ab, spill_idx, spill_cap);
	}
	if (ctx->still.active && !ctx->still.resolved) ctx->still.setup_d = d;
	else
	NH_LAUNCH(ctx, "adjacency_simple", k_adj_simple, nh_grid_for(B, 256, 4096), 256, st, B, ctx->deg, reinterpret_cast<const unsigned long long*>(ctx->deg + 2u * NH_DEG_STRIDE(B)), ctx->deg + 4u * NH_DEG_STRIDE(B), slot_key,
	          d->body_class, bodies->properties, bodies->momentum, d->simple, ctx->body_rec, ctx->body_pos, ctx->sort_seeded ? ctx->sort_sorted_idx : (const uint32_t*)nullptr);
	if (ctx->hint_capacity < B) {
		ctx->hint_capacity = 0;
		{ int rc = nh_device_buffers(ctx, { { &ctx->hint, sizeof(uint32_t) * (size_t)B } }); if (rc) return rc; }
		NH_HIP_CHECK(ctx, hipMemsetAsync(ctx->hint, 0xFF, sizeof(uint32_t) * (size_t)B, ctx->stream));
		ctx->hint_capacity = B;
	}
	d->cont.contacts = *contacts;
	d->cont.cursor = cursor; d->cont.pred_a = pred_a; d->cont.pred_b = pred_b; d->cont.level = level; d->cont.slot_key = slot_key;
	d->cont.level_hist = level_hist; d->cont.level_cursor = level_cursor; d->cont.tmp = tmp; d->cont.tent = tent;
	d->has_static8 = d->has_staticN = d->has_late = false; d->static_inert = false; d->general_lists = true;
	d->finish_pending = true;
	d->setup_pending = true; d->imp = imp; d->bodies_at_setup = *bodies;
	imp->consumed = true;
	ctx->pending = d;
	*out = d;
	return NH_OK;
}

int nh_still_abandon(nh_context* ctx) {
	nh_StillStep& ss = ctx->still;
	if (!ss.active || ss.resolved || ss.replaying) return NH_OK;
	nh_ContactConstraintData* d = ss.setup_d;
	ss.setup_d = nullptr;
	int rc = nh_still_undo_drops(ctx);
	if (rc) return rc;
	rc = nh_still_export_cache(ctx);
	if (rc) return rc;
	ss.contacts_stale = false;
	rc = nh_still_collide_again(ctx);
	if (rc) return rc;
	if (d) {
		const uint32_t B = d->body_count;
		NH_LAUNCH(ctx, "adjacency_simple", k_adj_simple, nh_grid_for(B, 256, 4096), 256, ctx->d_state, B, ctx->deg, reinterpret_cast<const unsigned long long*>(ctx->deg + 2u * NH_DEG_STRIDE(B)),
		          ctx->deg + 4u * NH_DEG_STRIDE(B), (const uint32_t*)nullptr, d->body_class, d->bodies_at_setup.properties, d->bodies_at_setup.momentum, d->simple,
		          ctx->body_rec, ctx->body_pos, ctx->sort_seeded ? ctx->sort_sorted_idx : (const uint32_t*)nullptr);
	}
	return NH_OK;
}
```

nudge_amd/csrc/nh_solve.hip:

```cpp
#include "nh_internal.h"
#include <type_traits>
#include <atomic>
#include <string.h>
#include "nh_solver.h"
#include "nh_narrowphase.h"

__global__ __launch_bounds__(256) void k_gravity(const nh_DevState* __restrict__ st, const uint32_t* __restrict__ active, nh_BodyMomentum* __restrict__ momentum,
                                                 float gx_dt, float gy_dt, float gz_dt, float damping) {
	uint32_t n = st->active;
	for (uint32_t k = blockIdx.x * blockDim.x + threadIdx.x; k < n; k += gridDim.x * blockDim.x) {
		uint32_t i = active[k];
		nh_BodyMomentum m = momentum[i];
		nh_gravity_damping(m.velocity, m.angular_velocity, gx_dt, gy_dt, gz_dt, damping);
		momentum[i] = m;
	}
}

__global__ __launch_bounds__(256) void k_advance(const nh_DevState* __restrict__ st, const uint32_t* __restrict__ active, nh_Transform* __restrict__ xf,
                                                 const nh_BodyMomentum* __restrict__ momentum, uint8_t* __restrict__ idle, float time_step) {
	uint32_t n = st->active;
	for (uint32_t k = blockIdx.x * blockDim.x + threadIdx.x; k < n; k += gridDim.x * blockDim.x) {
		uint32_t i = active[k];
		nh_Transform t = xf[i];
		nh_BodyMomentum m = momentum[i];
// ... 1613 lines not shown
	for (uint32_t x = tid + (tid == 0 ? T : 0u); x < nbodies; x += T) {
		reinterpret_cast<float4*>(momentum + x)[0] = s_m0[x]; reinterpret_cast<float4*>(momentum + x)[1] = s_m1[x];
	}
}

__global__ __launch_bounds__(256) void k_update_impulses(const nh_DevState* __restrict__ st, const uint32_t* __restrict__ order, const float4* __restrict__ rows4, size_t stride,
                                                         const float4* __restrict__ gstates, nh_CachedContactImpulse* __restrict__ out, const uint32_t* __restrict__ colour,
                                                         const uint2* __restrict__ gpair, uint32_t packed_end = 0u) {
	uint32_t n = st->general_contacts;
	for (uint32_t k = blockIdx.x * blockDim.x + threadIdx.x; k < n; k += gridDim.x * blockDim.x) {
		nh_state s;
		if (k < packed_end) { const float* ps = reinterpret_cast<const float*>(gstates) + 3 * (size_t)k; s.normal = ps[0]; s.friction_x = ps[1]; s.friction_y = ps[2]; }
		else { const float4 sv = gstates[k]; s.normal = sv.x; s.friction_x = sv.y; s.friction_y = sv.z; }
		float ox, oy, oz;
		if (gpair[k].x & NH_RADIAL_BIT) {
			nh_rowr r;
			load_rowr_soa(rows4, stride, k, r);
			nh_export_impulse_r(r, s, ox, oy, oz);
		} else {
			nh_row r;
			load_row_soa(rows4, stride, k, r);
			nh_export_impulse(r, s, ox, oy, oz);
		}
		const uint32_t c = order[k];
		*reinterpret_cast<float4*>(out + c) = make_float4(ox, oy, oz, colour ? __uint_as_float(colour[c]) : 0.0f);
	}
}

#include "nh_blocks.h"

extern "C" int nh_apply_gravity_damping(nh_context* ctx, const nh_ActiveBodies* active_bodies, const nh_BodyData* bodies,
                                        float time_step, const float gravity[3], float damping_rate) {
	if (!ctx || !active_bodies || !bodies || !gravity) return NH_ERR_INVALID;
	const bool follows_collide = ctx->gravity_may_overlap, after_collide = ctx->after_collide;
	const bool in_sequence = ctx->still.active && !ctx->still.resolved && after_collide && !ctx->pending && bodies->momentum == ctx->still.bodies.momentum &&
	                         active_bodies->indices == ctx->still.lay_active;
	{ int rc = nh_flush_pending(ctx, false, in_sequence); if (rc) return rc; }
	float damping = 1.0f - time_step * damping_rate;
	if ((ctx->flags & NH_FLAG_FUSED_STEP) && after_collide) {
		ctx->grav.pending = true;
		ctx->grav.gx_dt = gravity[0] * time_step; ctx->grav.gy_dt = gravity[1] * time_step; ctx->grav.gz_dt = gravity[2] * time_step;
		ctx->grav.damping = damping; ctx->grav.time_step = time_step;
		ctx->grav.active = active_bodies->indices; ctx->grav.momentum = bodies->momentum; ctx->grav.body_count = bodies->count;
		return NH_OK;
	}
	const bool overlap = follows_collide && ctx->side != nullptr;
	hipStream_t main_stream = ctx->stream;
	if (overlap) { NH_HIP_CHECK(ctx, hipStreamWaitEvent(ctx->side, ctx->ev_active, 0)); ctx->stream = ctx->side; }
	NH_LAUNCH(ctx, "gravity_damping", k_gravity, nh_grid_for(bodies->count, 256, 2048), 256, ctx->d_state, active_bodies->indices, bodies->momentum,
	          gravity[0] * time_step, gravity[1] * time_step, gravity[2] * time_step, damping);
	if (overlap) {
		ctx->stream = main_stream;
		NH_HIP_CHECK(ctx, hipEventRecord(ctx->ev_gravity, ctx->side));
		NH_HIP_CHECK(ctx, hipStreamWaitEvent(main_stream, ctx->ev_gravity, 0));
	}
	return NH_OK;
}

extern "C" int nh_advance(nh_context* ctx, const nh_ActiveBodies* active_bodies, const nh_BodyData* bodies, float time_step) {
	if (!ctx || !active_bodies || !bodies) return NH_ERR_INVALID;
	{ int rc = nh_flush_pending(ctx); if (rc) return rc; }
	ctx->advance_count++;
	if (ctx->adv.done) {
		ctx->adv.done = false;
		if (nh_asuint(time_step) != nh_asuint(ctx->adv.time_step)) return NH_ERR_INVALID;
		if (ctx->adv.rest)
			NH_LAUNCH(ctx, "advance_rest", k_advance_rest, nh_grid_for(bodies->count, 256, 2048), 256, ctx->d_state, active_bodies->indices, ctx->adv.body_class, bodies->transforms,
			          bodies->momentum, bodies->idle_counters, time_step);
		return ctx->stream_state.every ? nh_stream_after_advance(ctx) : NH_OK;
	}
	NH_LAUNCH(ctx, "advance", k_advance, nh_grid_for(bodies->count, 256, 2048), 256, ctx->d_state, active_bodies->indices, bodies->transforms,
	          bodies->momentum, bodies->idle_counters, time_step);
	return ctx->stream_state.every ? nh_stream_after_advance(ctx) : NH_OK;
}

static void ensure_csr(nh_context* ctx, nh_ContactConstraintData* d) {
	if (d->csr_ready) return;
	d->csr_ready = true;
	const uint32_t B = d->body_count;
	nh_scan_u32(ctx, ctx->deg, d->body_off, &ctx->d_state->pad0, B + 1, d->cont.tmp, nullptr);
	NH_LAUNCH(ctx, "adjacency_from_simple", k_adj_from_simple, nh_grid_for(B, 256, 4096), 256, B, d->body_class, d->body_off, d->simple, d->adj);
}

static int blk_reserve(nh_context* ctx, uint32_t B, uint32_t kcap) {
	nh_BlkBuffers& k = ctx->blk;
	if (!k.tables) {
		const size_t nb = NH_BLK_MAX_BLOCKS + 8u, nbins = (size_t)(NH_BLK_MAX_BLOCKS + 1u) * NH_BLK_MAX_COLOURS + 8u;
		NH_HIP_CHECK(ctx, hipMalloc((void**)&k.blk_count, sizeof(uint32_t) * nb));
		NH_HIP_CHECK(ctx, hipMalloc((void**)&k.own_base, sizeof(uint32_t) * nb));
		NH_HIP_CHECK(ctx, hipMalloc((void**)&k.bins, sizeof(uint32_t) * nbins));
		NH_HIP_CHECK(ctx, hipMalloc((void**)&k.bin_off, sizeof(uint32_t) * nbins));
		NH_HIP_CHECK(ctx, hipMalloc((void**)&k.ghost_base, sizeof(uint32_t) * nb));
		NH_HIP_CHECK(ctx, hipMalloc((void**)&k.ghost_count, sizeof(uint32_t) * nb));
// ... 411 lines not shown
	nh_CacheView cv = { nullptr, nullptr, nullptr, nullptr, nullptr, ctx->d_state };
	if (FUSED) { cv.tags = d->imp->tags; cv.features = d->imp->features; cv.ctags = d->imp->ctags; cv.cfeatures = d->imp->cfeatures; cv.cdata = d->imp->cdata; }
	if (d->static_inert) {
		const uint32_t grid = nh_grid_for(d->body_count, 256, 8192), flags = (FUSED && drop_states) ? 2u : 0u;
		if (!early4_done || d->has_late)
			launch_one_body<4, FUSED>(ctx, "solve_one_body", grid, d, bodies, iterations, cv, { d->contact_data, early4_done ? NH_CLS_STATIC4_LATE : NH_CLS_STATIC4, NH_CLS_STATIC4_LATE, flags, nullptr, nh_FusedStep(), nh_StillView(), nh_AheadView() });
		if (d->has_static8)
			launch_one_body<8, FUSED>(ctx, "solve_one_body8", grid, d, bodies, iterations, cv, { d->contact_data, NH_CLS_STATIC8, NH_CLS_STATIC8_LATE, flags, nullptr, nh_FusedStep(), nh_StillView(), nh_AheadView() });
	} else {
		launch_static<4, FUSED>(ctx, "apply_static", d, bodies, iterations, cv, NH_CLS_STATIC4, NH_CLS_STATIC4_LATE);
		if (d->has_static8) launch_static<8, FUSED>(ctx, "apply_static8", d, bodies, iterations, cv, NH_CLS_STATIC8, NH_CLS_STATIC8_LATE);
	}
	if (d->has_staticN && iterations) launch_static<0, false>(ctx, "apply_staticN", d, bodies, iterations, cv, NH_CLS_STATICN, NH_CLS_STATICN);
}
static int settle_gravity(nh_context* ctx) {
	if (!ctx->grav.pending) return NH_OK;
	ctx->grav.pending = false;
	NH_LAUNCH(ctx, "gravity_damping", k_gravity, nh_grid_for(ctx->grav.body_count, 256, 2048), 256, ctx->d_state, ctx->grav.active, ctx->grav.momentum, ctx->grav.gx_dt, ctx->grav.gy_dt, ctx->grav.gz_dt, ctx->grav.damping);
	return NH_OK;
}

static bool still_usable(const nh_context* ctx, const nh_ContactConstraintData* d, const nh_BodyData* bodies, uint32_t iterations, bool applied, bool from_apply, bool drop_states) {
	return applied && from_apply && drop_states && iterations != 0u && d->finish_pending && ctx->still.setup_d == d && ctx->grav.pending && ctx->grav.momentum == bodies->momentum && bodies->idle_counters &&
	       bodies->momentum == ctx->still.bodies.momentum && bodies->transforms == ctx->still.bodies.transforms && d->imp->cdata == ctx->still.cache_data && ctx->still.slots_current;
}
static inline bool still_reports_itself(const nh_StillStep& ss) { return ss.pipelined && ss.h_ring[0]; }
static nh_AheadView still_ahead_view(const nh_context* ctx) {
	const nh_ColliderData& cd = ctx->still.colliders;
	const uint32_t C = cd.boxes.count + cd.spheres.count;
	const uint8_t* gen = (C < (1u << NH_GEN_SHIFT) && !ctx->env_no_incremental) ? ctx->fat_gen : (const uint8_t*)nullptr;
	return { ctx->body_col, cd.boxes.transforms, cd.boxes.data, cd.spheres.transforms, cd.spheres.data, cd.boxes.count, ctx->own_xf, ctx->own_aabb_min, ctx->own_aabb_max, ctx->fat_box, ctx->fat_pairs, ctx->fat_pair_capacity,
	         ctx->lay_capacity, ctx->sort_keys_by_position, ctx->own_ctag, gen, ctx->rec, ctx->raw_data, ctx->raw_feature, ctx->cnt_sorted, ctx->still_delta, ctx->pair_list_capacity, C > (2u << 20) ? 1u : 0u };
}
static int still_solve(nh_context* ctx, nh_ContactConstraintData* d, const nh_BodyData* bodies, uint32_t iterations) {
	nh_StillStep& ss = ctx->still;
	const uint32_t B = d->body_count, grid = (B + 63u) / 64u;
	const nh_CacheView cv = { nullptr, nullptr, nullptr, nullptr, reinterpret_cast<const nh_CachedContactImpulse*>(ctx->sc_imp), ctx->d_state };
	const nh_StillView sv = { ctx->body_rec, ctx->body_pos, ctx->cnt_sorted, ctx->start_sorted, ctx->raw_feature, ctx->sc_feat, ctx->sc_count, ctx->lay_capacity, ctx->still_delta, ctx->step_parity };
	nh_FusedStep fs = fused_gravity(ctx);
	fs.bits = 3u | (ss.sleepers ? 4u : 0u) | ((ss.sleepers && !ss.no_sleeper_skip) ? 8u : 0u); fs.idle = bodies->idle_counters; fs.seq = ctx->collide_seq;
	fs.ghost_first = ctx->halo_ghost_first; fs.host_counters = still_reports_itself(ss) ? reinterpret_cast<uint32_t*>(ss.h_ring[ctx->collide_seq & 1u]) : nullptr;
	fs.guard_seq = ss.verdict.pending ? ss.verdict.seq : ctx->collide_seq;
	ctx->halo_split.launched = false;
	const bool ahead = ss.ahead_plain && ss.more_steps && ss.ahead_map_ok && !ss.no_ahead && !ss.ahead_world_bad && ctx->own_xf && ctx->body_col && ctx->body_col_capacity >= B;
	const bool pair = ahead && !ss.no_pair && !ss.pair_world_bad && ss.pair_owned_seq != 0u && ctx->pair_list && ctx->fat_pairs && ctx->own_ctag &&
	                  (uint64_t)ss.colliders.boxes.count + ss.colliders.spheres.count < (1ull << 31);
	const nh_AheadView av = ahead ? still_ahead_view(ctx) : nh_AheadView();
	const bool split = pair && ctx->halo_split.armed && ss.early_verdict && ss.steps_left > 0u && !ctx->timing && ctx->halo_split.bound != 0u;
	auto with = [&](const nh_FusedStep& f) { return nh_OneBodyLaunch{ ctx->raw_data, NH_CLS_STATIC4, NH_CLS_STATIC4, 2u, d->simple, f, sv, av }; };
	if (split) {
		nh_FusedStep fi = fs, fb = fs;
		fi.part = 2u; fi.xskip = ctx->halo_split.mask;
		fb.part = 1u; fb.xlist = ctx->halo_split.list; fb.xcount = ctx->halo_split.count; fb.host_counters = nullptr;
		launch_one_body<4, true, true, 1, true, true, true, true>(ctx, "solve_still", grid, d, bodies, iterations, cv, with(fi));
		NH_HIP_CHECK(ctx, hipStreamWaitEvent(ctx->halo_split.stream, ss.ev_ring[0], 0));
		launch_one_body<4, true, true, 1, true, true, true, true>(ctx, nullptr, (ctx->halo_split.bound + 63u) / 64u, d, bodies, iterations, cv, with(fb), ctx->halo_split.stream);
		ctx->halo_split.launched = true;
	} else if (pair) launch_one_body<4, true, true, 1, true, true, true>(ctx, "solve_still", grid, d, bodies, iterations, cv, with(fs));
	else if (ahead) launch_one_body<4, true, true, 1, true, true>(ctx, "solve_still", grid, d, bodies, iterations, cv, with(fs));
	else launch_one_body<4, true, true, 1, true>(ctx, "solve_still", grid, d, bodies, iterations, cv, with(fs));
	ss.ahead_ready = ahead; ss.pair_ready = pair;
	return NH_OK;
}
static inline bool still_held(const nh_DevState* h, uint32_t seq) { return h->still_failed_seq < seq && h->error == 0u; }
static void adopt_counters(nh_context* ctx, const nh_DevState* h, uint32_t seq, uint32_t parity, uint64_t collide_mark) {
	ctx->still.confirmed_seq = seq;
	if (h != ctx->h_state) memcpy(ctx->h_state, h, NH_COUNTER_WORDS * sizeof(uint32_t));
	if (!ctx->idle_unknown) { ctx->idle_bound = (int)h->max_idle[parity]; ctx->idle_bound_mark = collide_mark; }
	nh_still_note_movers(ctx, h, seq);
}
static int still_verdict(nh_context* ctx, bool* confirmed) {
	nh_StillStep& ss = ctx->still;
	if (still_reports_itself(ss)) {
		if (ss.verdict.pending) {
			if (ss.verdict.event) NH_HIP_CHECK(ctx, hipEventSynchronize(ss.ev_ring[ss.verdict.slot]));
			else { const int w = nh_still_await_number(ctx); if (w) return w == 2 ? NH_ERR_HIP : NH_INTERNAL_STILL_FAILED; }
			const nh_DevState* h = ss.h_ring[ss.verdict.slot];
			if (!still_held(h, ss.verdict.seq)) return NH_INTERNAL_STILL_FAILED;
			adopt_counters(ctx, h, ss.verdict.seq, ss.verdict.parity, ss.verdict.collide_mark);
			ss.verdict.pending = false;
		}
		const int slot = (int)(ctx->collide_seq & 1u);
		const bool ring_event = ctx->halo_split.launched || ctx->no_early_counts;
		if (ring_event) NH_HIP_CHECK(ctx, hipEventRecord(ss.ev_ring[slot], ctx->stream));
		ss.verdict.event = ring_event;
		ss.verdict.pending = true; ss.verdict.seq = ctx->collide_seq; ss.verdict.parity = ctx->step_parity; ss.verdict.slot = slot; ss.verdict.collide_mark = ctx->collide_mark;
		*confirmed = true;
	} else if (ss.early_verdict) {
		ss.early_verdict = false;
		NH_HIP_CHECK(ctx, hipEventSynchronize(ss.ev_ring[0]));
		const nh_DevState* h = ss.h_ring[0];
		*confirmed = still_held(h, ctx->collide_seq);
		if (*confirmed) {
			adopt_counters(ctx, h, ctx->collide_seq, ctx->step_parity, ctx->collide_mark);
// ... 51 lines not shown
		}
		if (confirmed) { still_confirmed(ctx, d); return NH_OK; }
		{ int rc = nh_still_abandon(ctx); if (rc) return rc; }
	}
	if (!d->finish_pending) { int rc = settle_gravity(ctx); if (rc) return rc; }
	if (d->finish_pending) {
		int rc = speculative_launch(ctx, d, bodies, iterations, from_apply, drop_states);
		if (rc) return rc;
		early4_done = d->static_inert;
	}
	launch_apply_static<true>(ctx, d, bodies, iterations, early4_done, drop_states);
	return NH_OK;
}

int nh_flush_pending(nh_context* ctx, bool keep_gravity, bool in_sequence) {
	if (!in_sequence) { int rc = nh_still_abandon(ctx); if (rc) return rc; }
	ctx->gravity_may_overlap = false;
	ctx->after_collide = false;
	nh_ContactConstraintData* d = ctx->pending;
	if (d) {
		ctx->pending = nullptr;
		if (d->setup_pending) {
			d->setup_pending = false;
			int rc = first_apply(ctx, d, &d->bodies_at_setup, 0);
			if (rc) return rc;
			if (d->general_contacts && d->blk.active && d->blk.warm_pending) { d->blk.warm_pending = false; blk_run(ctx, d, &d->bodies_at_setup, true, 0u); }
		}
	}
	return keep_gravity ? NH_OK : settle_gravity(ctx);
}

extern "C" int nh_apply_impulses(nh_context* ctx, nh_ContactConstraintData* d, const nh_BodyData* bodies, uint32_t iterations) {
	if (!ctx || !d || !bodies) return NH_ERR_INVALID;
	if (ctx->pending && ctx->pending != d) { int rc = nh_flush_pending(ctx); if (rc) return rc; }
	if (ctx->still.active && !ctx->still.resolved && !(ctx->pending == d && d->setup_pending)) { int rc = nh_still_abandon(ctx); if (rc) return rc; }
	ctx->gravity_may_overlap = false; ctx->after_collide = false;
	const bool first = d->setup_pending;
	if (!first && !d->states_kept) return NH_ERR_INVALID;
	d->setup_pending = false;
	ctx->pending = nullptr;
	if (first) { int rc = first_apply(ctx, d, bodies, iterations, true); if (rc) return rc; }
	else { int rc = settle_gravity(ctx); if (rc) return rc; launch_apply_static<false>(ctx, d, bodies, iterations, false); }
	if (d->general_contacts && d->blk.active) {
		const bool warm = d->blk.warm_pending;
		d->blk.warm_pending = false;
		blk_run(ctx, d, bodies, warm, iterations);
	} else if (d->general_contacts && (d->resident || d->resident_bodies)) {
		if (iterations) launch_resident(ctx, d, bodies, d->levels, nullptr, iterations, 0u);
	} else if (d->general_contacts) for (uint32_t it = 0; it < iterations; ++it) launch_levels<false>(ctx, d, bodies, nullptr);
	return NH_OK;
}

extern "C" int nh_update_cached_impulses(nh_context* ctx, nh_ContactConstraintData* d, nh_ContactImpulseData* imp) {
	if (!ctx || !d || !imp) return NH_ERR_INVALID;
	{ int rc = nh_flush_pending(ctx); if (rc) return rc; }
	if (d->general_contacts)
		NH_LAUNCH(ctx, "update_impulses", k_update_impulses, nh_grid_for(d->general_contacts, 256, 4096), 256, ctx->d_state, d->level_order, (const float4*)d->rows, (size_t)d->contact_capacity,
		          (const float4*)d->gstates, imp->data, (ctx->flags & NH_FLAG_EXACT_ORDER) ? (const uint32_t*)nullptr : (const uint32_t*)((d->blk.active && d->blk.local) ? d->cont.tent : d->cont.level), d->gpair,
		          d->blk.active ? d->blk.res_off[0] : 0u);
	return NH_OK;
}
```

nudge_amd/csrc/nh_step.hip:

```cpp
#include "nh_internal.h"
#include <atomic>
#include <chrono>
#include <string.h>

void nh_still_note_movers(nh_context* ctx, const nh_DevState* h, uint32_t seq) {
	nh_StillStep& ss = ctx->still;
	if (ss.sleepers && h->active == 0u) ss.ok_next = false;
	if (seq != 0u) { if (h->active == ss.sleep_last_active) { if (ss.sleep_stable < 0xffffu) ss.sleep_stable++; } else { ss.sleep_stable = 0u; ss.sleep_last_active = h->active; } }
	if (ss.pair_owned_seq != 0u && seq >= ss.pair_owned_seq) { if (h->pair_unowned > ctx->pair_list_capacity) ss.pair_world_bad = true; else { ss.pair_world_ok = true; ss.pair_listed = h->pair_unowned; } }
	if (h->ahead_multi) ss.ahead_world_bad = true;
	if (h->fat_inserts != ss.seen_inserts) ss.movers_left = 16u;
	else if (ss.movers_left) ss.movers_left--;
	ss.seen_inserts = h->fat_inserts; ss.seen_rebuilds = h->fat_rebuilds;
}

__global__ __launch_bounds__(256) void k_view_sleep_keys(const nh_DevState* __restrict__ st, const nh_Record* __restrict__ rec, const uint64_t* __restrict__ rec_key, uint64_t* __restrict__ out) {
	const uint32_t n = st->records;
	for (uint32_t r = blockIdx.x * blockDim.x + threadIdx.x; r < n; r += gridDim.x * blockDim.x) out[r] = (rec[r].count & NH_REC_SLEEPING) ? rec_key[r] : ~0ull;
}
__global__ __launch_bounds__(256) void k_view_sleep_copy(nh_DevState* __restrict__ st, const uint64_t* __restrict__ sorted, uint64_t* __restrict__ out, uint32_t capacity) {
	const uint32_t n = st->sleeping;
	if (n > capacity) { if (blockIdx.x == 0 && threadIdx.x == 0) st->error = NH_ERR_CONTACT_CAPACITY; return; }
	for (uint32_t i = blockIdx.x * blockDim.x + threadIdx.x; i < n; i += gridDim.x * blockDim.x) out[i] = sorted[i];
}
// ... 76 lines not shown
			else if (now - t0 > std::chrono::milliseconds(2)) {
				const hipError_t q = hipStreamQuery(ctx->stream);
				if (q == hipSuccess) { if (*flag == ss.verdict.seq) break; return 1; }
				if (q != hipErrorNotReady) { ctx->last_hip_error = (int)q; return 2; }
			}
		}
		__builtin_ia32_pause();
	}
	std::atomic_thread_fence(std::memory_order_acquire);
	ctx->early_reads++;
	return 0;
}

int nh_still_verdict_now(nh_context* ctx) {
	nh_StillStep& ss = ctx->still;
	if (!ss.verdict.pending) return 0;
	const nh_DevState* h = ss.h_ring[ss.verdict.slot];
	if (ss.verdict.event) {
		const hipError_t e = hipEventSynchronize(ss.ev_ring[ss.verdict.slot]);
		if (e != hipSuccess) { ss.verdict.pending = false; ctx->last_hip_error = (int)e; return 2; }
	} else {
		const int w = nh_still_await_number(ctx);
		if (w) { ss.verdict.pending = false; return w; }
	}
	ss.verdict.pending = false;
	if (h->still_failed_seq >= ss.verdict.seq || h->error) return 1;
	ss.confirmed_seq = ss.verdict.seq;
	memcpy(ctx->h_state, h, NH_COUNTER_WORDS * sizeof(uint32_t));
	if (!ctx->idle_unknown) { ctx->idle_bound = (int)h->max_idle[ss.verdict.parity]; ctx->idle_bound_mark = ss.verdict.collide_mark; }
	nh_still_note_movers(ctx, h, ss.verdict.seq);
	return 0;
}

static int still_forget_failed(nh_context* ctx, bool advanced, uint32_t voided) {
	nh_StillStep& ss = ctx->still;
	ss.verdict.pending = false;
	ss.active = false; ss.resolved = false; ss.setup_d = nullptr; ss.ok_next = false; ss.ahead_ready = false; ss.own_current = false;
	ss.note_failure();
	if (ss.sleepers) {
		if (ss.sleep_backoff_len < 8u || ss.sleep_run >= 32u) ss.sleep_backoff_len = 8u; else if (ss.sleep_backoff_len < 64u) ss.sleep_backoff_len *= 2u;
		ss.sleep_backoff = ss.sleep_backoff_len; ss.sleep_stable = 0u; ss.sleep_run = 0u;
	}
	ss.failed += voided;
	ctx->pending = nullptr;
	ctx->grav.pending = false; ctx->grav.rest_pending = false; ctx->adv.done = false;
	ctx->after_collide = false; ctx->gravity_may_overlap = false;
	if (advanced && ctx->advance_count) ctx->advance_count--;
	if (advanced) nh_stream_void_advance(ctx);
	{ int rc = nh_still_undo_drops(ctx); if (rc) return rc; }
	return nh_still_export_cache(ctx);
}

static bool same_bodies_arrays(const nh_BodyData& a, const nh_BodyData& b) {
	return a.transforms == b.transforms && a.properties == b.properties && a.momentum == b.momentum && a.idle_counters == b.idle_counters && a.count == b.count;
}
static bool same_collider_arrays(const nh_ColliderData& a, const nh_ColliderData& b) {
	return a.boxes.tags == b.boxes.tags && a.boxes.data == b.boxes.data && a.boxes.transforms == b.boxes.transforms && a.boxes.count == b.boxes.count &&
	       a.spheres.tags == b.spheres.tags && a.spheres.data == b.spheres.data && a.spheres.transforms == b.spheres.transforms && a.spheres.count == b.spheres.count;
}

extern "C" int nh_step(nh_context* ctx, const nh_StepArgs* a, uint32_t steps) {
	if (!ctx || !a || !a->active_bodies || !a->contacts || !a->bodies || !a->colliders || !a->contact_cache) return NH_ERR_INVALID;
	NH_HIP_CHECK(ctx, hipSetDevice(ctx->device));
	nh_StillStep& ss = ctx->still;
	if (!ss.h_ring[0] && !ss.ring_failed) {
		for (int k = 0; k < 2; ++k) {
			if (hipHostMalloc((void**)&ss.h_ring[k], sizeof(nh_DevState), 0) != hipSuccess || hipEventCreateWithFlags(&ss.ev_ring[k], hipEventDisableTiming) != hipSuccess) { ss.ring_failed = true; break; }
			memset(ss.h_ring[k], 0, sizeof(nh_DevState));
		}
		if (ss.ring_failed) {
			for (int k = 0; k < 2; ++k) {
				if (ss.h_ring[k]) { (void)hipHostFree(ss.h_ring[k]); ss.h_ring[k] = nullptr; }
				if (ss.ev_ring[k]) { (void)hipEventDestroy(ss.ev_ring[k]); ss.ev_ring[k] = nullptr; }
			}
		}
	}
	ss.pipelined = ss.h_ring[0] != nullptr && (ctx->flags & NH_FLAG_FUSED_STEP) && !(ctx->flags & (NH_FLAG_SYNC_COUNTS | NH_FLAG_EXACT_ORDER)) && !ss.disabled &&
	               !(ctx->timing && ctx->timing_filter.empty()) &&
	               !ctx->step_hook;
	ss.verdict.pending = false;
	ss.ahead_map_ok = false; ss.ahead_ready = false;
	int result = NH_OK;
	uint32_t i = 0;
	while (i < steps || ss.verdict.pending) {
		if (i >= steps) {
			const int v = nh_still_verdict_now(ctx);
			if (v == 0) break;
			if (v == 2) { result = NH_ERR_HIP; break; }
			{ int rc = still_forget_failed(ctx, true, 1u); if (rc) { result = rc; break; } }
			i -= 1;
			continue;
		}
		if (ctx->asleep.streak >= 2u && !ctx->asleep.disabled && !ctx->step_hook && !ss.verdict.pending && !ctx->pending && (ctx->flags & NH_FLAG_FUSED_STEP) && !(ctx->flags & NH_FLAG_SYNC_COUNTS) && !ctx->timing &&
		    same_bodies_arrays(*a->bodies, ss.lay_bodies) && same_collider_arrays(*a->colliders, ss.lay_colliders) && a->contacts->data == ss.lay_contacts.data && a->contacts->tags == ss.lay_contacts.tags &&
		    a->contacts->sleeping_pairs == ss.lay_contacts.sleeping_pairs && a->active_bodies->indices == ss.lay_active && a->contact_cache->data == ss.cache_data && a->contact_cache->tags == ss.cache_tags && a->contact_cache->features == ss.cache_features) {
			const int v = nh_asleep_verify(ctx, a->bodies, a->colliders);
			if (v < 0) { result = -v; break; }
			if (v == 0) { ss.sleep_backoff = ss.sleep_backoff > steps - i ? ss.sleep_backoff - (steps - i) : 0u; ctx->asleep.steps += steps - i; if (ctx->stream_state.every) ctx->stream_state.advances += steps - i; i = steps; continue; }
			ctx->asleep.streak = 0;
		}
		int rc;
		if (ctx->step_hook && (rc = ctx->step_hook(ctx, ctx->step_hook_user, i))) { result = rc; break; }
		ss.more_steps = i + 1u < steps; ss.steps_left = steps - 1u - i; ss.substep = i;
		nh_Arena temporary = a->arena;
		nh_ContactImpulseData* imp = nullptr;
		nh_ContactConstraintData* con = nullptr;
		if ((rc = nh_collide(ctx, a->active_bodies, a->contacts, a->bodies, a->colliders, a->body_connections, temporary)) ||
		    (rc = nh_apply_gravity_damping(ctx, a->active_bodies, a->bodies, a->time_step, a->gravity, a->damping_rate)) ||
		    (rc = nh_read_cached_impulses(ctx, a->contact_cache, a->contacts, &temporary, &imp)) ||
		    (rc = nh_setup_contact_constraints(ctx, a->active_bodies, a->contacts, a->bodies, imp, &temporary, &con)) ||
		    (rc = nh_apply_impulses(ctx, con, a->bodies, a->iterations))) {
			if (rc == NH_INTERNAL_STILL_FAILED && i > 0) {
				{ int rc2 = still_forget_failed(ctx, true, ctx->still.active ? 2u : 1u); if (rc2) { result = rc2; break; } }
				i -= 1;
				continue;
			}
			result = rc == NH_INTERNAL_STILL_FAILED ? NH_ERR_INVALID : rc;
			break;
		}
		if ((rc = nh_update_cached_impulses(ctx, con, imp)) || (rc = nh_write_cached_impulses(ctx, a->contact_cache, a->contacts, imp)) ||
		    (rc = nh_advance(ctx, a->active_bodies, a->bodies, a->time_step))) { result = rc; break; }
		++i;
	}
	ss.pipelined = false; ss.more_steps = false; ss.ahead_ready = false; ss.ahead_map_ok = false; ss.steps_left = 0u; ss.substep = 0u; ss.own_current = false;
	if (result && ss.verdict.pending) { if (ss.verdict.event) hipEventSynchronize(ss.ev_ring[ss.verdict.slot]); else hipStreamSynchronize(ctx->stream); ss.verdict.pending = false; }
	return result;
}
```

nudge_amd/engine.py:

```python
from __future__ import annotations

import ctypes as C
import os
import subprocess
import warnings

import numpy as np

from . import scenes as S

_HERE = os.path.dirname(os.path.abspath(__file__))
_LIB_PATH = os.environ.get("NUDGE_HIP_LIBRARY") or os.path.join(_HERE, "libnudge_hip.so")
_LIB = None

NH_FLAG_SYNC_COUNTS = 1
NH_FLAG_EXACT_ORDER = 2
NH_FLAG_SINGLE_APPLY = 4
NH_FLAG_FUSED_STEP = 8
NH_VIEW_CONTACTS, NH_VIEW_CACHE, NH_VIEW_ACTIVE, NH_VIEW_ALL = 1, 2, 4, 7
OPTION_NAMES = ("no_still", "no_kept_pairs", "no_incremental", "no_sort_reuse", "sort_radix", "bucket_tile", "bucket_target",
                "colour_check_seeds", "no_resident", "no_blocks", "blk_check", "blk_min", "blk_target", "blk_rows_global",
                "blk_global_colours", "blk_profile", "no_asleep", "no_blk_chain", "no_local_still", "no_xform_ahead", "sync_exports_views", "no_pair_ahead", "no_sleeper_skip", "halo_overlap", "no_early_counts", "no_sleeper_ahead", "no_listed_lookup")

EXPORTS = [
    "nh_create", "nh_destroy", "nh_set_flags", "nh_synchronize", "nh_read_counts", "nh_export_views", "nh_set_cache_count",
    "nh_set_tag_bits", "nh_set_pair_capacity", "nh_set_option", "nh_bodies_changed", "nh_error_string", "nh_last_hip_error", "nh_collide", "nh_apply_gravity_damping",
    "nh_read_cached_impulses", "nh_write_cached_impulses", "nh_setup_contact_constraints", "nh_apply_impulses",
    "nh_update_cached_impulses", "nh_advance", "nh_contact_impulses_device", "nh_enable_timing", "nh_set_timing_filter", "nh_kernel_times",
    "nh_halo_pack", "nh_halo_unpack", "nh_halo_update", "nh_append_contacts", "nh_step", "nh_stream_state", "nh_stream_latest",
    "nh_partition_create", "nh_partition_destroy", "nh_partition_info", "nh_partition_pack_migrants", "nh_partition_unpack_migrants", "nh_partition_pack_ghosts",
    "nh_partition_top_speed", "nh_partition_set_peer_speeds", "nh_partition_refresh_is_quiet", "nh_partition_mark_ghosts", "nh_partition_pack_deltas", "nh_partition_unpack_deltas",
    "nh_partition_pack_momentum", "nh_partition_unpack_momentum", "nh_partition_exchange_iteration", "nh_partition_unpack_ghosts", "nh_partition_pack_step", "nh_partition_unpack_step", "nh_partition_choose_cut", "nh_partition_set_cut",
    "nh_partition_set_transport", "nh_partition_exchange_step", "nh_partition_step", "nh_partition_transport_check", "nh_partition_transport_result", "nh_set_first_ghost_body",
    "nh_query_build", "nh_query_refit", "nh_query_stats", "nh_raycast", "nh_overlap", "nh_penetration", "nh_spherecast", "nh_raycast_all", "nh_spherecast_all", "nh_boxcast_all", "nh_capsulecast_all", "nh_boxcast", "nh_capsulecast", "nh_closest", "nh_closest_k", "nh_distance", "nh_move",
    "nh_raycast_k", "nh_spherecast_k", "nh_boxcast_k", "nh_capsulecast_k",
    "nh_query_set_layers", "nh_query_filter", "nh_query_layer_info",
]
HALO_RECORD_BYTES = 64


class Arena(C.Structure):
    _fields_ = [("data", C.c_void_p), ("size", C.c_size_t)]


class ContactData(C.Structure):
    _fields_ = [("data", C.c_void_p), ("bodies", C.c_void_p), ("tags", C.c_void_p), ("features", C.c_void_p),
                ("capacity", C.c_uint32), ("count", C.c_uint32), ("sleeping_pairs", C.c_void_p), ("sleeping_count", C.c_uint32)]


class _Shapes(C.Structure):
    _fields_ = [("tags", C.c_void_p), ("data", C.c_void_p), ("transforms", C.c_void_p), ("count", C.c_uint32)]


class ColliderData(C.Structure):
    _fields_ = [("boxes", _Shapes), ("spheres", _Shapes)]


class BodyData(C.Structure):
    _fields_ = [("transforms", C.c_void_p), ("properties", C.c_void_p), ("momentum", C.c_void_p),
                ("idle_counters", C.c_void_p), ("count", C.c_uint32)]


class BodyConnections(C.Structure):
    _fields_ = [("data", C.c_void_p), ("count", C.c_uint32)]


class ContactCache(C.Structure):
    _fields_ = [("tags", C.c_void_p), ("features", C.c_void_p), ("data", C.c_void_p), ("capacity", C.c_uint32), ("count", C.c_uint32)]


class ActiveBodies(C.Structure):
    _fields_ = [("indices", C.c_void_p), ("capacity", C.c_uint32), ("count", C.c_uint32)]


class Counts(C.Structure):
    _fields_ = [(n, C.c_uint32) for n in ("colliders", "pairs", "contacts", "sleeping_pairs", "active_bodies", "cache", "culled",
                                          "large_colliders", "general_contacts", "levels", "error", "has_other_bodies", "unleveled", "raw_pairs", "broadphase_rebuilds", "sort_reuses", "broadphase_inserts",
                                          "still_steps", "still_replays", "still_diff_key", "still_diff_count", "still_diff_feature", "still_diff_escape",
                                          "blk_blocks", "blk_bodies", "blk_ghosts", "asleep_steps", "ahead_steps", "fused_steps", "pair_steps", "pair_diag_roles", "pair_diag_record", "pair_diag_scale", "pair_diag_owned")]

    def as_dict(self):
        return {n: int(getattr(self, n)) for n, _ in self._fields_}


class StepArgs(C.Structure):
    _fields_ = [("active_bodies", C.POINTER(ActiveBodies)), ("contacts", C.POINTER(ContactData)), ("bodies", C.POINTER(BodyData)), ("colliders", C.POINTER(ColliderData)),
                ("body_connections", C.POINTER(BodyConnections)), ("contact_cache", C.POINTER(ContactCache)), ("arena", Arena),
                ("time_step", C.c_float), ("gravity", C.c_float * 3), ("damping_rate", C.c_float), ("iterations", C.c_uint32)]


class PartitionConfig(C.Structure):
    _fields_ = [("rank", C.c_uint32), ("ranks", C.c_uint32), ("lo", C.c_double), ("hi", C.c_double), ("n_owned", C.c_uint32), ("n_static_box", C.c_uint32), ("n_static_sph", C.c_uint32),
                ("body_capacity", C.c_uint32), ("box_capacity", C.c_uint32), ("sphere_capacity", C.c_uint32), ("epoch", C.c_uint32),
                ("time_step", C.c_double), ("gravity", C.c_double), ("speed_floor", C.c_double), ("max_reach", C.c_double), ("cut_slack", C.c_double)]


class PartitionInfo(C.Structure):
    _fields_ = [("n_owned", C.c_uint32), ("n_bodies", C.c_uint32), ("n_boxes", C.c_uint32), ("n_spheres", C.c_uint32), ("ghost_out", C.c_uint32 * 2), ("ghost_in", C.c_uint32 * 2),
                ("lo", C.c_double), ("hi", C.c_double), ("migrated_out", C.c_uint64), ("migrated_in", C.c_uint64), ("refreshes", C.c_uint64), ("cut_moves", C.c_uint64), ("quiet_refreshes", C.c_uint64)]


class QueryStats(C.Structure):
    _fields_ = [("colliders", C.c_uint32), ("run_length", C.c_uint32), ("runs", C.c_uint32), ("top_nodes", C.c_uint32), ("top_depth", C.c_uint32)]


class QueryLayerInfo(C.Structure):
    _fields_ = [("set", C.c_uint32), ("colliders", C.c_uint32), ("any_layers", C.c_uint32), ("reserved", C.c_uint32)]


class Ray(C.Structure):
    _fields_ = [("origin", C.c_float * 3), ("max_t", C.c_float), ("direction", C.c_float * 3), ("ignore_body", C.c_uint32)]

# ... 941 lines not shown
```

Measured before the change: 3937.

## Carry ahead-computed pair contacts across nh_step calls into the next call

At the last substep of a pipelined nh_step call, the solve kernel now computes the next step's pair/contact data ahead of time into separate carry buffers. The next call adopts them by swapping raw contact buffers and running a check kernel that verifies the collider transforms match. This extends the existing within-call ahead/pair pipelining across call boundaries, so the first step of each call can skip collision work. In exchange it adds extra buffers, invalidation hooks on every API entry point, and a failure path that syncs the host and backs off.

```diff
diff --git a/include/nudge_hip.h b/include/nudge_hip.h
--- a/include/nudge_hip.h
+++ b/include/nudge_hip.h
@@ -106,6 +106,8 @@
 	uint32_t fused_steps;
 	uint32_t pair_steps;
 	uint32_t pair_diag[4];
+	uint32_t carry_steps;
+	uint32_t carry_failed;
 } nh_Counts;
 
 int nh_create(nh_context** out, int device, void* stream, uint32_t flags);
diff --git a/nudge_amd/csrc/nh_append.hip b/nudge_amd/csrc/nh_append.hip
--- a/nudge_amd/csrc/nh_append.hip
+++ b/nudge_amd/csrc/nh_append.hip
@@ -82,6 +82,7 @@
 extern "C" int nh_append_contacts(nh_context* ctx, nh_ContactData* contacts, const nh_BodyData* bodies, uint32_t extra, uint32_t* positions, nh_Arena temporary) {
 	if (!ctx || !contacts || !bodies) return NH_ERR_INVALID;
 	if (!extra) return NH_OK;
+	nh_carry_drop(ctx);
 	if (extra > 65536u || extra > contacts->capacity) return NH_ERR_INVALID;
 	if (ctx->setup_seq == ctx->collide_seq || !ctx->deg) return NH_ERR_STALE_SETUP;
 	{ int rc = nh_flush_pending(ctx); if (rc) return rc; }
diff --git a/nudge_amd/csrc/nh_cache.hip b/nudge_amd/csrc/nh_cache.hip
--- a/nudge_amd/csrc/nh_cache.hip
+++ b/nudge_amd/csrc/nh_cache.hip
@@ -181,6 +181,7 @@
 
 extern "C" int nh_read_cached_impulses(nh_context* ctx, const nh_ContactCache* cache, const nh_ContactData* contacts, nh_Arena* memory, nh_ContactImpulseData** out) {
 	if (!ctx || !cache || !contacts || !memory || !out) return NH_ERR_INVALID;
+	nh_carry_drop_outside_step(ctx);
 	{
 		const nh_StillStep& ss = ctx->still;
 		const bool in_sequence = ss.active && !ss.resolved && !ctx->pending && cache->tags == ss.cache_tags && cache->features == ss.cache_features && cache->data == ss.cache_data &&
@@ -239,6 +240,7 @@
 
 extern "C" int nh_write_cached_impulses(nh_context* ctx, nh_ContactCache* cache, const nh_ContactData* contacts, nh_ContactImpulseData* imp) {
 	if (!ctx || !cache || !contacts || !imp) return NH_ERR_INVALID;
+	nh_carry_drop_outside_step(ctx);
 	{ int rc = nh_flush_pending(ctx); if (rc) return rc; }
 	{
 		nh_StillStep& ss = ctx->still;
diff --git a/nudge_amd/csrc/nh_collide.hip b/nudge_amd/csrc/nh_collide.hip
--- a/nudge_amd/csrc/nh_collide.hip
+++ b/nudge_amd/csrc/nh_collide.hip
@@ -1293,6 +1293,42 @@
 	if (__ballot(changed) != 0ull && lane == 0) atomicMax(&st->still_failed_seq, seq);
 }
 
+__global__ __launch_bounds__(256) void k_carry_check(nh_DevState* __restrict__ st, uint32_t seq, uint32_t parity, const nh_Transform* __restrict__ body_xf, uint32_t nbodies,
+                                                     const nh_Transform* __restrict__ box_xf, uint32_t nbox, const nh_Transform* __restrict__ sph_xf, uint32_t nsph, const nh_xform* __restrict__ own_xf,
+                                                     const int2* __restrict__ delta, const uint32_t* __restrict__ carry_cnt, uint32_t* __restrict__ cnt_sorted, nh_Record* __restrict__ rec,
+                                                     const uint32_t* __restrict__ sorted_idx, uint32_t pair_cap) {
+	if (blockIdx.x == 0) {
+		const uint32_t listed = st->delta_overflow[parity] ? 0u : min(st->delta_count[parity], NH_DELTA_MAX);
+		for (uint32_t k = threadIdx.x; k < listed; k += blockDim.x) {
+			const uint32_t pos = (uint32_t)delta[parity * NH_DELTA_MAX + k].x;
+			if (pos >= pair_cap) continue;
+			const uint32_t count = carry_cnt[pos], r = sorted_idx[pos];
+			cnt_sorted[pos] = count;
+			if (r < pair_cap) rec[r].count = count;
+		}
+	}
+	bool differs = false;
+	const uint32_t n = nbox + nsph;
+	for (uint32_t c = blockIdx.x * blockDim.x + threadIdx.x; c < n; c += gridDim.x * blockDim.x) {
+		const nh_Transform l = c < nbox ? box_xf[c] : sph_xf[c - nbox];
+		const float4* const on_file = reinterpret_cast<const float4*>(own_xf) + 2u * (size_t)c;
+		const float4 w0 = on_file[0], w1 = on_file[1];
+		if (l.body >= nbodies) { differs = true; continue; }
+		const nh_Transform b = body_xf[l.body];
+		const nh_quat bq = { b.rotation[0], b.rotation[1], b.rotation[2], b.rotation[3] };
+		const nh_quat lq = { l.rotation[0], l.rotation[1], l.rotation[2], l.rotation[3] };
+		const nh_f3 p = nh_rotate(bq, nh_make3(l.position[0], l.position[1], l.position[2])) + nh_make3(b.position[0], b.position[1], b.position[2]);
+		const nh_quat q = nh_qmul(bq, lq);
+		differs |= __float_as_uint(p.x) != __float_as_uint(w0.x) || __float_as_uint(p.y) != __float_as_uint(w0.y) || __float_as_uint(p.z) != __float_as_uint(w0.z) || l.body != __float_as_uint(w0.w) ||
+		           __float_as_uint(q.x) != __float_as_uint(w1.x) || __float_as_uint(q.y) != __float_as_uint(w1.y) || __float_as_uint(q.z) != __float_as_uint(w1.z) || __float_as_uint(q.s) != __float_as_uint(w1.w);
+	}
+	if (__ballot(differs) != 0ull && nh_lane() == 0) { atomicMax(&st->still_failed_seq, seq); st->carry_failed_seq = seq; atomicAdd(&st->still_diff[3], 1u); }
+}
+__global__ void k_carry_reset(nh_DevState* __restrict__ st, uint32_t parity) {
+	if (threadIdx.x == 0) { st->delta_count[parity] = 0u; st->delta_overflow[parity] = 0u; }
+	for (uint32_t k = threadIdx.x; k < NH_AHEAD_PARTS * 8u; k += blockDim.x) (&st->ahead_part[parity][0][0])[k] = (k & 7u) < 3u ? 0xffffffffu : 0u;
+}
+
 __global__ __launch_bounds__(256) void k_asleep_check(nh_DevState* __restrict__ st, const nh_Transform* __restrict__ body_xf, const uint8_t* __restrict__ idle, uint32_t nbodies,
                                                       const nh_Transform* __restrict__ box_xf, const nh_BoxCollider* __restrict__ box_data, const uint32_t* __restrict__ box_tags, uint32_t nbox,
                                                       const nh_Transform* __restrict__ sph_xf, const nh_SphereCollider* __restrict__ sph_data, const uint32_t* __restrict__ sph_tags, uint32_t nsph,
@@ -1638,6 +1674,7 @@
                           const nh_BodyData* bodies, const nh_ColliderData* colliders,
                           const nh_BodyConnections* body_connections, nh_Arena temporary) {
 	if (!ctx || !active_bodies || !contacts || !bodies || !colliders) return NH_ERR_INVALID;
+	nh_carry_drop_outside_step(ctx);
 	NH_HIP_CHECK(ctx, hipSetDevice(ctx->device));
 	{ int rc = nh_flush_pending(ctx); if (rc) return rc; }
 	nh_StillStep& ss = ctx->still;
@@ -1783,6 +1820,8 @@
 static int reserve_pair_layout(nh_context* ctx, uint32_t pair_cap, uint32_t cap, bool* fresh) {
 	if (ctx->lay_capacity == pair_cap && ctx->lay_contact_capacity == cap) return NH_OK;
 	ctx->lay_capacity = 0; ctx->lay_contact_capacity = 0;
+	nh_carry_drop(ctx); ctx->carry_capacity = 0; ctx->carry_slots = 0;
+	{ int rc = nh_device_buffers(ctx, { { &ctx->carry_raw_data, 0 }, { &ctx->carry_raw_feature, 0 }, { &ctx->carry_cnt, 0 }, { &ctx->carry_rec, 0 } }); if (rc) return rc; }
 	const size_t slots = (size_t)4 * pair_cap + cap, cache_slots = (size_t)5 * pair_cap + 64u, pairs = pair_cap;
 	ctx->pair_list_capacity = pair_cap / 8u + 1024u;
 	{ int rc = nh_device_buffers(ctx, { { &ctx->raw_data, sizeof(nh_Contact) * slots }, { &ctx->raw_feature, sizeof(uint32_t) * slots + 64u }, { &ctx->rec, sizeof(nh_Record) * pairs + 64u },
@@ -1811,7 +1850,7 @@
 	ctx->own_capacity = 0;
 	{ int rc = nh_device_buffers(ctx, { { &ctx->own_xf, sizeof(nh_xform) * (size_t)C + 64u }, { &ctx->own_aabb_min, sizeof(float4) * (size_t)C + 64u }, { &ctx->own_aabb_max, sizeof(float4) * (size_t)C + 64u },
 	                                    { &ctx->own_ctag, sizeof(uint32_t) * (size_t)C + 64u } }); if (rc) return rc; }
-	ctx->own_capacity = C; ctx->still.ahead_ready = false; ctx->still.own_current = false;
+	ctx->own_capacity = C; ctx->still.ahead_ready = false; ctx->still.own_current = false; nh_carry_drop(ctx);
 	return NH_OK;
 }
 
@@ -1823,6 +1862,7 @@
 	bool take_map;
 	bool list_unowned;
 	bool early_verdict;
+	bool carry_step;
 	bool delta_scan;
 	bool local;
 	uint32_t sleeper_skip;
@@ -1840,16 +1880,26 @@
 	ss.was_sleepers = sleepers;
 	const bool sleep_stable = sleepers && !ss.no_sleeper_ahead && !ss.no_pair && ss.sleep_stable >= 4u && ss.sleep_backoff == 0u && !ctx->step_hook && ss.pipelined && C <= (2u << 20);
 	const bool plain = !movers && (!sleepers || sleep_stable) && !ss.appended_pairs && (nbox >= 2 || nsph != 0u);
+	if (ss.carry_adopt && !(plain && !sleepers && ss.ahead_ready && ss.pair_ready && !ss.no_ahead && !ss.no_pair && ctx->carry_raw_data && ctx->carry_capacity == ctx->lay_capacity)) {
+		ss.carry_adopt = false; ss.ahead_ready = false; ss.pair_ready = false;
+		hipLaunchKernelGGL(k_carry_reset, dim3(1), dim3(256), 0, ctx->stream, ctx->d_state, ctx->step_parity);
+	}
 	const bool ahead_step = f.ahead_step = plain && ss.ahead_ready && !ss.no_ahead && (!sleepers || ss.pair_ready);
 	ss.ahead_ready = false; ss.ahead_plain = plain;
 	const bool pair_step = f.pair_step = ahead_step && ss.pair_ready && !ss.no_pair;
 	ss.pair_ready = false; ss.pair_step = pair_step; ss.early_verdict = false;
-	if (pair_step) ss.pair_steps++;
+	const bool carry_step = f.carry_step = ss.carry_step = pair_step && ss.carry_adopt;
+	ss.carry_adopt = false;
+	if (carry_step) { ss.carry_steps++; ss.carry_seq = ctx->collide_seq; if (ss.carry_run < 0xffffu) ss.carry_run++; if (ss.carry_run >= 256u) ss.carry_backoff = 0u; }
+	if (pair_step && !carry_step) ss.pair_steps++;
 	if (pair_step && sleepers && ss.sleep_run < 0xffffu) ss.sleep_run++;
-	if (ahead_step) ss.ahead_steps++;
+	if (ahead_step && !carry_step) ss.ahead_steps++;
 	f.sleeper_skip = (sleepers && ss.substep > 0u && ss.own_current && !ctx->step_hook && !ss.no_sleeper_skip) ? 1u : 0u;
 	if (sleepers && !ahead_step) ss.ahead_map_ok = false;
-	f.take_map = !ahead_step && plain && ss.more_steps && !ss.no_ahead && !ss.ahead_world_bad && !ss.ahead_map_ok && c.bodies->idle_counters;
+	ss.carry_launch = !ss.more_steps && plain && !sleepers && ss.pipelined && !ss.no_carry && !ss.no_ahead && !ss.no_pair && !ss.pair_world_bad && !ss.ahead_world_bad && !ctx->halo_split.armed && !ctx->step_hook && C <= (2u << 20) &&
+	                  (pair_step || ss.substep == 0u) && ss.calls_steady >= 2u && ss.good_run >= 4u && c.bodies->idle_counters;
+	if (ss.carry_launch && ss.carry_hold) { ss.carry_hold--; ss.carry_launch = false; }
+	f.take_map = !ahead_step && plain && (ss.more_steps || ss.carry_launch) && !ss.no_ahead && !ss.ahead_world_bad && !ss.ahead_map_ok && c.bodies->idle_counters;
 	f.list_unowned = f.take_map && ss.pair_owned_seq == 0u && !ss.no_pair && ctx->pair_mark;
 	f.delta_scan = C > (2u << 20) || (sleepers && !pair_step);
 	if (sleepers) ss.undo_dirty = true;
@@ -1899,6 +1949,11 @@
 		NH_LAUNCH(ctx, "reinsert_still", k_reinsert, 256, 256, st, nbox, ctx->grid_sbox, ctx->grid_cstart, ctx->grid_large, ctx->fat_box, ctx->fat_gen, ctx->fat_esc_mark, ctx->fat_esc_list,
 		          ctx->fat_moved_list, ctx->collide_seq, ctx->fat_pairs, ctx->fat_pair_capacity, 1u, ctx->step_parity, C, ctx->body_rec, pair_cap);
 	const uint8_t* gen = m.incremental ? ctx->fat_gen : (const uint8_t*)nullptr;
+	if (f.carry_step) {
+		std::swap(ctx->raw_data, ctx->carry_raw_data); std::swap(ctx->raw_feature, ctx->carry_raw_feature);
+		NH_LAUNCH(ctx, "carry_check", k_carry_check, nh_grid_for(C, 256, 2048), 256, st, ctx->collide_seq, ctx->step_parity, bodies->transforms, B, colliders->boxes.transforms, nbox, colliders->spheres.transforms, nsph,
+		          xf, ctx->still_delta, ctx->carry_cnt, ctx->cnt_sorted, ctx->rec, ctx->sort_sorted_idx, pair_cap);
+	}
 	if (f.pair_step) {
 		const uint32_t pair_waves = ss.pair_world_ok ? std::min(std::max((ss.pair_listed + 63u) / 64u, 1u), 127u) : 127u;
 		NH_LAUNCH(ctx, "pair_begin", k_pair_begin, 1u + pair_waves, 64, st, ctx->step_parity, ctx->collide_seq, ctx->pair_list, ctx->pair_list_capacity, ctx->fat_pairs, ctx->fat_pair_capacity, pair_cap, gen,
@@ -2069,6 +2124,8 @@
 	{ int rc = reserve_body_layout(ctx, c.B, &lay_fresh); if (rc) return rc; }
 	nh_StillStep& ss = ctx->still;
 	if (lay_fresh) { ss.slots_current = false; ss.ok_next = false; }
+	if (ss.carry_out && !(ss.carry_out == 1u && ss.carry_adopt && want_still)) { ss.carry_adopt = false; ss.ahead_ready = false; hipLaunchKernelGGL(k_carry_reset, dim3(1), dim3(256), 0, ctx->stream, ctx->d_state, ctx->step_parity); }
+	ss.carry_out = 0u;
 	if (!same_colliders(*colliders, ss.lay_colliders)) ss.ahead_world_bad = false;
 	ss.lay_bodies = *bodies; ss.lay_colliders = *colliders; ss.lay_contacts = *contacts; ss.lay_active = active_bodies->indices; ss.lay_active_capacity = active_bodies->capacity;
 	ss.appended = false;
@@ -2077,6 +2134,7 @@
 	if (may_sleep && sleepers_ok) { int rc = reserve_one(ctx, &ctx->still_awake, &ctx->still_awake_capacity, c.B, (size_t)c.B + 64u); if (rc) return rc; }
 	const bool still = want_still && (c.no_islands || sleepers_ok) && !m.bp_direct && !m.drop_kept && !m.drop_sort_order && !lay_fresh && ctx->sort_seeded && !ctx->env_sort_radix &&
 	                   !ctx->env_no_sort_reuse && c.C != 0u;
+	if (!still && ss.carry_adopt) { ss.carry_adopt = false; hipLaunchKernelGGL(k_carry_reset, dim3(1), dim3(256), 0, ctx->stream, ctx->d_state, ctx->step_parity); }
 	if (!still) return full_step(ctx, c, s, m);
 	{ int rc = reserve_own(ctx, c.C); if (rc) return rc; }
 	const StillForm f = still_decide(ctx, c, m);
diff --git a/nudge_amd/csrc/nh_context.hip b/nudge_amd/csrc/nh_context.hip
--- a/nudge_amd/csrc/nh_context.hip
+++ b/nudge_amd/csrc/nh_context.hip
@@ -53,6 +53,7 @@
 	ctx->blk.target = 900u;
 	ctx->raw_data = nullptr; ctx->raw_feature = nullptr; ctx->raw_slots = 0; ctx->rec = nullptr; ctx->lay_rank = nullptr; ctx->cnt_sorted = nullptr; ctx->start_sorted = nullptr; ctx->dense_slot = nullptr;
 	ctx->sc_imp = nullptr; ctx->sc_feat = nullptr; ctx->sc_count = nullptr; ctx->sc_undo = nullptr; ctx->pair_mark = nullptr; ctx->pair_list = nullptr; ctx->pair_list_capacity = 0; ctx->exp_cnt = nullptr; ctx->exp_start = nullptr; ctx->exp_scan_tmp = nullptr; ctx->still_delta = nullptr; ctx->lay_capacity = 0; ctx->lay_contact_capacity = 0;
+	ctx->carry_raw_data = nullptr; ctx->carry_raw_feature = nullptr; ctx->carry_cnt = nullptr; ctx->carry_rec = nullptr; ctx->carry_capacity = 0; ctx->carry_slots = 0;
 	ctx->own_xf = nullptr; ctx->own_aabb_min = nullptr; ctx->own_aabb_max = nullptr; ctx->own_ctag = nullptr; ctx->own_capacity = 0; ctx->body_col = nullptr; ctx->body_col_capacity = 0;
 	ctx->still_awake = nullptr; ctx->still_awake_capacity = 0; ctx->exp_sleep_a = nullptr; ctx->exp_sleep_b = nullptr; ctx->exp_sleep_hist = nullptr; ctx->exp_flags = nullptr; ctx->exp_sleep_capacity = 0; ctx->exp_flags_capacity = 0;
 	ctx->lay_class = nullptr; ctx->lay_simple = nullptr; ctx->body_rec = nullptr; ctx->body_pos = nullptr; ctx->lay_body_capacity = 0;
@@ -106,7 +107,7 @@
 		                 ctx->fat_esc_mark, ctx->fat_esc_list, ctx->fat_moved_list, ctx->sort_keys_by_position, ctx->sort_sorted_keys, ctx->sort_sorted_idx, ctx->sort_splitters, ctx->sort_counts, ctx->sort_starts,
 		                 ctx->raw_data, ctx->raw_feature, ctx->rec, ctx->lay_rank, ctx->cnt_sorted, ctx->start_sorted, ctx->dense_slot, ctx->sc_imp, ctx->sc_feat, ctx->sc_count, ctx->sc_undo, ctx->pair_mark, ctx->pair_list, ctx->exp_cnt, ctx->exp_start,
 		                 ctx->exp_scan_tmp, ctx->still_delta, ctx->lay_class, ctx->lay_simple, ctx->body_rec, ctx->body_pos, ctx->still_awake, ctx->exp_sleep_a, ctx->exp_sleep_b, ctx->exp_sleep_hist, ctx->exp_flags,
-		                 ctx->own_xf, ctx->own_aabb_min, ctx->own_aabb_max, ctx->own_ctag, ctx->body_col };
+		                 ctx->own_xf, ctx->own_aabb_min, ctx->own_aabb_max, ctx->own_ctag, ctx->body_col, ctx->carry_raw_data, ctx->carry_raw_feature, ctx->carry_cnt, ctx->carry_rec };
 		for (void* b : bufs) if (b) hipFree(b);
 	}
 	{
@@ -122,6 +123,7 @@
 
 extern "C" int nh_set_flags(nh_context* ctx, uint32_t flags) {
 	if (!ctx) return NH_ERR_INVALID;
+	nh_carry_drop(ctx);
 	{ int rc = nh_flush_pending(ctx); if (rc) return rc; }
 	ctx->asleep.streak = 0;
 	ctx->flags = (flags & NH_FLAG_FUSED_STEP) ? (flags | NH_FLAG_SINGLE_APPLY) : flags;
@@ -129,6 +131,7 @@
 }
 extern "C" int nh_set_first_ghost_body(nh_context* ctx, uint32_t first_ghost) {
 	if (!ctx) return NH_ERR_INVALID;
+	nh_carry_drop(ctx);
 	{ int rc = nh_flush_pending(ctx); if (rc) return rc; }
 	ctx->asleep.streak = 0;
 	ctx->first_ghost = first_ghost;
@@ -137,6 +140,7 @@
 
 extern "C" int nh_set_option(nh_context* ctx, const char* name, int value) {
 	if (!ctx || !name) return NH_ERR_INVALID;
+	nh_carry_drop(ctx);
 	{ int rc = nh_flush_pending(ctx); if (rc) return rc; }
 	const std::string n(name);
 	const bool on = value != 0;
@@ -151,6 +155,7 @@
 	else if (n == "no_pair_ahead") ctx->still.no_pair = on;
 	else if (n == "no_xform_ahead") ctx->still.no_ahead = on;
 	else if (n == "no_local_still") ctx->still.no_local = on;
+	else if (n == "no_carry") ctx->still.no_carry = on;
 	else if (n == "no_still") ctx->still.disabled = on;
 	else if (n == "sort_radix") ctx->env_sort_radix = on;
 	else if (n == "no_sort_reuse") ctx->env_no_sort_reuse = on;
@@ -174,11 +179,12 @@
 	return NH_OK;
 }
 
-extern "C" int nh_set_tag_bits(nh_context* ctx, uint32_t bits) { if (!ctx || bits < 1 || bits > 32) return NH_ERR_INVALID; ctx->tag_bits = bits; return NH_OK; }
+extern "C" int nh_set_tag_bits(nh_context* ctx, uint32_t bits) { if (!ctx || bits < 1 || bits > 32) return NH_ERR_INVALID; nh_carry_drop(ctx); ctx->tag_bits = bits; return NH_OK; }
 
 extern "C" int nh_bodies_changed(nh_context* ctx) {
 	if (!ctx) return NH_ERR_INVALID;
 	{ int rc = nh_still_abandon(ctx); if (rc) return rc; }
+	nh_carry_drop(ctx); ctx->still.carry_hold = 0u; ctx->still.carry_backoff = 0u;
 	ctx->idle_bound = -1; ctx->idle_unknown = true;
 	ctx->asleep.streak = 0;
 	ctx->still.ok_next = false;
@@ -187,7 +193,7 @@
 	return NH_OK;
 }
 
-extern "C" int nh_set_pair_capacity(nh_context* ctx, uint32_t pairs) { if (!ctx) return NH_ERR_INVALID; ctx->pair_capacity = pairs; return NH_OK; }
+extern "C" int nh_set_pair_capacity(nh_context* ctx, uint32_t pairs) { if (!ctx) return NH_ERR_INVALID; nh_carry_drop(ctx); ctx->pair_capacity = pairs; return NH_OK; }
 
 extern "C" int nh_synchronize(nh_context* ctx) {
 	if (!ctx) return NH_ERR_INVALID;
@@ -209,6 +215,7 @@
 	out->still_steps = (uint32_t)(ctx->still.launched - ctx->still.failed - ((ctx->still.active && !ctx->still.resolved) ? 1u : 0u)); out->still_replays = (uint32_t)ctx->still.failed;
 	for (int k = 0; k < 4; ++k) out->still_diff[k] = h->still_diff[k];
 	out->asleep_steps = (uint32_t)ctx->asleep.steps; out->ahead_steps = (uint32_t)ctx->still.ahead_steps; out->fused_steps = 0u; out->pair_steps = (uint32_t)ctx->still.pair_steps;
+	out->carry_steps = (uint32_t)ctx->still.carry_steps; out->carry_failed = (uint32_t)ctx->still.carry_failed;
 	for (int k = 0; k < 4; ++k) out->pair_diag[k] = h->pair_diag[k];
 	out->blk_blocks = h->blk.nblk; out->blk_bodies = h->blk.bodies; out->blk_ghosts = h->blk.ghost_cursor;
 	out->has_other_bodies = h->has_other; out->broadphase_rebuilds = h->fat_rebuilds; out->sort_reuses = h->sort_reuses; out->broadphase_inserts = h->fat_inserts; out->unleveled = h->unleveled; out->raw_pairs = h->pairs + h->pairs_sph;
@@ -230,6 +237,7 @@
 extern "C" int nh_set_cache_count(nh_context* ctx, uint32_t count) {
 	if (!ctx) return NH_ERR_INVALID;
 	{ int rc = nh_still_abandon(ctx); if (rc) return rc; }
+	nh_carry_drop(ctx);
 	ctx->asleep.streak = 0;
 	ctx->still.cache_ok = false; ctx->still.slots_current = false; ctx->still.cache_stale = false;
 	hipLaunchKernelGGL(k_set_cache_count, dim3(1), dim3(1), 0, ctx->stream, ctx->d_state, count);
@@ -354,6 +362,7 @@
 
 extern "C" int nh_enable_timing(nh_context* ctx, int on) {
 	if (!ctx) return NH_ERR_INVALID;
+	nh_carry_drop(ctx);
 	hipStreamSynchronize(ctx->stream);
 	if (ctx->timing) nh_timer_collect(ctx);
 	ctx->timing = on != 0;
@@ -362,6 +371,7 @@
 
 extern "C" int nh_set_timing_filter(nh_context* ctx, const char* name) {
 	if (!ctx) return NH_ERR_INVALID;
+	nh_carry_drop(ctx);
 	ctx->timing_filter = name ? name : "";
 	return NH_OK;
 }
diff --git a/nudge_amd/csrc/nh_internal.h b/nudge_amd/csrc/nh_internal.h
--- a/nudge_amd/csrc/nh_internal.h
+++ b/nudge_amd/csrc/nh_internal.h
@@ -117,6 +117,7 @@
 	uint32_t still_static_min[3], still_static_max[3];
 	uint32_t ahead_part[2][64][8];
 	nh_BlkGrid blk;
+	uint32_t carry_failed_seq;
 };
 
 struct nh_TimerSlot { const char* name; hipEvent_t a, b; };
@@ -208,6 +209,16 @@
 	bool own_current;
 	bool views_sleepers;
 	bool sleep_pairs_current, active_current;
+	bool no_carry;
+	bool in_step;
+	uint32_t carry_out;
+	bool carry_adopt;
+	bool carry_step;
+	bool carry_launch;
+	uint32_t carry_seq;
+	uint32_t calls_steady;
+	uint32_t carry_hold, carry_backoff, carry_run;
+	uint64_t carry_steps, carry_failed;
 	void note_failure() { hold = (1u << fail_level) - 1u; if (fail_level < 6u) ++fail_level; good_run = 0; }
 	void note_confirmed() { if (++good_run >= 16u) fail_level = 0; }
 };
@@ -314,6 +325,7 @@
 	int2* still_delta;
 	uint32_t* exp_cnt; uint32_t* exp_start; uint32_t* exp_scan_tmp;
 	uint32_t lay_capacity, lay_contact_capacity;
+	nh_Contact* carry_raw_data; uint32_t* carry_raw_feature; uint32_t* carry_cnt; struct nh_Record* carry_rec; uint32_t carry_capacity, carry_slots;
 	uint8_t* lay_class; uint2* lay_simple; uint32_t* body_rec; uint32_t* body_pos; uint32_t lay_body_capacity;
 	nh_StillStep still;
 	int (*step_hook)(nh_context* ctx, void* user, uint32_t sub_step); void* step_hook_user; uint32_t halo_ghost_first;
@@ -342,6 +354,8 @@
 int nh_asleep_verify(nh_context* ctx, const nh_BodyData* bodies, const nh_ColliderData* colliders);
 int nh_still_collide_again(nh_context* ctx);
 int nh_still_view_contacts(nh_context* ctx);
+void nh_carry_drop(nh_context* ctx);
+static inline void nh_carry_drop_outside_step(nh_context* ctx) { if (!ctx->still.in_step) nh_carry_drop(ctx); }
 struct nh_ContactImpulseData;
 NH_LOCAL void nh_run_cull(nh_context* ctx, nh_ContactImpulseData* d, uint32_t sleeping_on_host);
 NH_LOCAL void nh_materialize_lookup(nh_context* ctx, nh_ContactImpulseData* d, const nh_BodyPair* bodies = nullptr, const uint8_t* body_class = nullptr, const uint32_t* general_list = nullptr, uint32_t general = 0u);
diff --git a/nudge_amd/csrc/nh_partition.hip b/nudge_amd/csrc/nh_partition.hip
--- a/nudge_amd/csrc/nh_partition.hip
+++ b/nudge_amd/csrc/nh_partition.hip
@@ -988,6 +988,7 @@
 
 static int halo_unpack(nh_context* ctx, const nh_BodyData* bodies, uint32_t first_slot, uint32_t count, const void* in, bool same_bodies) {
 	if (!ctx || !bodies || (count && !in) || (uint64_t)first_slot + count > bodies->count) return NH_ERR_INVALID;
+	nh_carry_drop(ctx);
 	{ int rc = nh_flush_pending(ctx); if (rc) return rc; }
 	if (count && !same_bodies) { ctx->idle_bound = -1; ctx->idle_unknown = true; }
 	if (count) NH_LAUNCH(ctx, "halo_unpack", k_halo_unpack, nh_grid_for(count, 256, 1024), 256, bodies->transforms, bodies->momentum, bodies->idle_counters, first_slot, count, (const nh_HaloRecord*)in);
diff --git a/nudge_amd/csrc/nh_schedule.hip b/nudge_amd/csrc/nh_schedule.hip
--- a/nudge_amd/csrc/nh_schedule.hip
+++ b/nudge_amd/csrc/nh_schedule.hip
@@ -210,6 +210,7 @@
 extern "C" int nh_setup_contact_constraints(nh_context* ctx, const nh_ActiveBodies* active_bodies, const nh_ContactData* contacts,
                                             const nh_BodyData* bodies, nh_ContactImpulseData* imp, nh_Arena* memory, nh_ContactConstraintData** out) {
 	if (!ctx || !contacts || !bodies || !imp || !memory || !out) return NH_ERR_INVALID;
+	nh_carry_drop_outside_step(ctx);
 	{
 		const nh_StillStep& ss = ctx->still;
 		const bool in_sequence = ss.active && !ss.resolved && !ctx->pending && contacts->data == ss.lay_contacts.data && contacts->bodies == ss.lay_contacts.bodies &&
@@ -288,6 +289,7 @@
 	if (!ss.active || ss.resolved || ss.replaying) return NH_OK;
 	nh_ContactConstraintData* d = ss.setup_d;
 	ss.setup_d = nullptr;
+	nh_carry_drop(ctx);
 	int rc = nh_still_undo_drops(ctx);
 	if (rc) return rc;
 	rc = nh_still_export_cache(ctx);
diff --git a/nudge_amd/csrc/nh_solve.hip b/nudge_amd/csrc/nh_solve.hip
--- a/nudge_amd/csrc/nh_solve.hip
+++ b/nudge_amd/csrc/nh_solve.hip
@@ -1669,6 +1669,7 @@
 extern "C" int nh_apply_gravity_damping(nh_context* ctx, const nh_ActiveBodies* active_bodies, const nh_BodyData* bodies,
                                         float time_step, const float gravity[3], float damping_rate) {
 	if (!ctx || !active_bodies || !bodies || !gravity) return NH_ERR_INVALID;
+	nh_carry_drop_outside_step(ctx);
 	const bool follows_collide = ctx->gravity_may_overlap, after_collide = ctx->after_collide;
 	const bool in_sequence = ctx->still.active && !ctx->still.resolved && after_collide && !ctx->pending && bodies->momentum == ctx->still.bodies.momentum &&
 	                         active_bodies->indices == ctx->still.lay_active;
@@ -1696,6 +1697,7 @@
 
 extern "C" int nh_advance(nh_context* ctx, const nh_ActiveBodies* active_bodies, const nh_BodyData* bodies, float time_step) {
 	if (!ctx || !active_bodies || !bodies) return NH_ERR_INVALID;
+	nh_carry_drop_outside_step(ctx);
 	{ int rc = nh_flush_pending(ctx); if (rc) return rc; }
 	ctx->advance_count++;
 	if (ctx->adv.done) {
@@ -2173,6 +2175,15 @@
 	return { ctx->body_col, cd.boxes.transforms, cd.boxes.data, cd.spheres.transforms, cd.spheres.data, cd.boxes.count, ctx->own_xf, ctx->own_aabb_min, ctx->own_aabb_max, ctx->fat_box, ctx->fat_pairs, ctx->fat_pair_capacity,
 	         ctx->lay_capacity, ctx->sort_keys_by_position, ctx->own_ctag, gen, ctx->rec, ctx->raw_data, ctx->raw_feature, ctx->cnt_sorted, ctx->still_delta, ctx->pair_list_capacity, C > (2u << 20) ? 1u : 0u };
 }
+static int carry_reserve(nh_context* ctx) {
+	if (ctx->carry_raw_data && ctx->carry_capacity == ctx->lay_capacity && ctx->carry_slots == ctx->raw_slots) return NH_OK;
+	ctx->carry_capacity = 0; ctx->carry_slots = 0;
+	const size_t slots = ctx->raw_slots, pairs = ctx->lay_capacity;
+	{ int rc = nh_device_buffers(ctx, { { &ctx->carry_raw_data, sizeof(nh_Contact) * slots }, { &ctx->carry_raw_feature, sizeof(uint32_t) * slots + 64u },
+	                                    { &ctx->carry_cnt, sizeof(uint32_t) * (pairs + 2u) }, { &ctx->carry_rec, sizeof(nh_Record) * pairs + 64u } }); if (rc) return rc; }
+	ctx->carry_capacity = ctx->lay_capacity; ctx->carry_slots = ctx->raw_slots;
+	return NH_OK;
+}
 static int still_solve(nh_context* ctx, nh_ContactConstraintData* d, const nh_BodyData* bodies, uint32_t iterations) {
 	nh_StillStep& ss = ctx->still;
 	const uint32_t B = d->body_count, grid = (B + 63u) / 64u;
@@ -2183,10 +2194,13 @@
 	fs.ghost_first = ctx->halo_ghost_first; fs.host_counters = still_reports_itself(ss) ? reinterpret_cast<uint32_t*>(ss.h_ring[ctx->collide_seq & 1u]) : nullptr;
 	fs.guard_seq = ss.verdict.pending ? ss.verdict.seq : ctx->collide_seq;
 	ctx->halo_split.launched = false;
-	const bool ahead = ss.ahead_plain && ss.more_steps && ss.ahead_map_ok && !ss.no_ahead && !ss.ahead_world_bad && ctx->own_xf && ctx->body_col && ctx->body_col_capacity >= B;
-	const bool pair = ahead && !ss.no_pair && !ss.pair_world_bad && ss.pair_owned_seq != 0u && ctx->pair_list && ctx->fat_pairs && ctx->own_ctag &&
-	                  (uint64_t)ss.colliders.boxes.count + ss.colliders.spheres.count < (1ull << 31);
-	const nh_AheadView av = ahead ? still_ahead_view(ctx) : nh_AheadView();
+	const bool pair_world = !ss.no_pair && !ss.pair_world_bad && ss.pair_owned_seq != 0u && ctx->pair_list && ctx->fat_pairs && ctx->own_ctag &&
+	                        (uint64_t)ss.colliders.boxes.count + ss.colliders.spheres.count < (1ull << 31);
+	const bool carry = !ss.more_steps && ss.carry_launch && pair_world && !ctx->halo_split.armed && carry_reserve(ctx) == NH_OK;
+	const bool ahead = ss.ahead_plain && (ss.more_steps || carry) && ss.ahead_map_ok && !ss.no_ahead && !ss.ahead_world_bad && ctx->own_xf && ctx->body_col && ctx->body_col_capacity >= B;
+	const bool pair = ahead && pair_world;
+	nh_AheadView av = ahead ? still_ahead_view(ctx) : nh_AheadView();
+	if (ahead && carry) { av.raw_data = ctx->carry_raw_data; av.raw_feature = ctx->carry_raw_feature; av.cnt_sorted = ctx->carry_cnt; av.rec = ctx->carry_rec; }
 	const bool split = pair && ctx->halo_split.armed && ss.early_verdict && ss.steps_left > 0u && !ctx->timing && ctx->halo_split.bound != 0u;
 	auto with = [&](const nh_FusedStep& f) { return nh_OneBodyLaunch{ ctx->raw_data, NH_CLS_STATIC4, NH_CLS_STATIC4, 2u, d->simple, f, sv, av }; };
 	if (split) {
@@ -2200,7 +2214,9 @@
 	} else if (pair) launch_one_body<4, true, true, 1, true, true, true>(ctx, "solve_still", grid, d, bodies, iterations, cv, with(fs));
 	else if (ahead) launch_one_body<4, true, true, 1, true, true>(ctx, "solve_still", grid, d, bodies, iterations, cv, with(fs));
 	else launch_one_body<4, true, true, 1, true>(ctx, "solve_still", grid, d, bodies, iterations, cv, with(fs));
-	ss.ahead_ready = ahead; ss.pair_ready = pair;
+	ss.ahead_ready = ahead && ss.more_steps; ss.pair_ready = pair && ss.more_steps;
+	ss.carry_out = (ahead && !ss.more_steps) ? 1u : 0u;
+	ss.carry_launch = false;
 	return NH_OK;
 }
 static inline bool still_held(const nh_DevState* h, uint32_t seq) { return h->still_failed_seq < seq && h->error == 0u; }
@@ -2318,6 +2334,7 @@
 
 extern "C" int nh_apply_impulses(nh_context* ctx, nh_ContactConstraintData* d, const nh_BodyData* bodies, uint32_t iterations) {
 	if (!ctx || !d || !bodies) return NH_ERR_INVALID;
+	nh_carry_drop_outside_step(ctx);
 	if (ctx->pending && ctx->pending != d) { int rc = nh_flush_pending(ctx); if (rc) return rc; }
 	if (ctx->still.active && !ctx->still.resolved && !(ctx->pending == d && d->setup_pending)) { int rc = nh_still_abandon(ctx); if (rc) return rc; }
 	ctx->gravity_may_overlap = false; ctx->after_collide = false;
@@ -2339,6 +2356,7 @@
 
 extern "C" int nh_update_cached_impulses(nh_context* ctx, nh_ContactConstraintData* d, nh_ContactImpulseData* imp) {
 	if (!ctx || !d || !imp) return NH_ERR_INVALID;
+	nh_carry_drop_outside_step(ctx);
 	{ int rc = nh_flush_pending(ctx); if (rc) return rc; }
 	if (d->general_contacts)
 		NH_LAUNCH(ctx, "update_impulses", k_update_impulses, nh_grid_for(d->general_contacts, 256, 4096), 256, ctx->d_state, d->level_order, (const float4*)d->rows, (size_t)d->contact_capacity,
diff --git a/nudge_amd/csrc/nh_step.hip b/nudge_amd/csrc/nh_step.hip
--- a/nudge_amd/csrc/nh_step.hip
+++ b/nudge_amd/csrc/nh_step.hip
@@ -132,9 +132,27 @@
 	return 0;
 }
 
+static void carry_void(nh_StillStep& ss) { if (ss.carry_out) ss.carry_out = 2u; ss.carry_adopt = false; }
+void nh_carry_drop(nh_context* ctx) { carry_void(ctx->still); ctx->still.calls_steady = 0u; }
+static int carry_note_failure(nh_context* ctx) {
+	nh_StillStep& ss = ctx->still;
+	if (ss.carry_seq == 0u || ss.carry_seq <= ss.confirmed_seq) return NH_OK;
+	uint32_t failed_seq = 0u;
+	NH_HIP_CHECK(ctx, hipMemcpyAsync(&failed_seq, &ctx->d_state->carry_failed_seq, sizeof(uint32_t), hipMemcpyDeviceToHost, ctx->stream));
+	NH_HIP_CHECK(ctx, hipStreamSynchronize(ctx->stream));
+	if (failed_seq == ss.carry_seq) ss.carry_failed++;
+	ss.carry_steps--;
+	ss.carry_seq = 0u; ss.carry_run = 0u;
+	ss.carry_backoff = 256u;
+	ss.carry_hold = ss.carry_backoff;
+	return NH_OK;
+}
+
 static int still_forget_failed(nh_context* ctx, bool advanced, uint32_t voided) {
 	nh_StillStep& ss = ctx->still;
 	ss.verdict.pending = false;
+	{ int rc = carry_note_failure(ctx); if (rc) return rc; }
+	nh_carry_drop(ctx);
 	ss.active = false; ss.resolved = false; ss.setup_d = nullptr; ss.ok_next = false; ss.ahead_ready = false; ss.own_current = false;
 	ss.note_failure();
 	if (ss.sleepers) {
@@ -179,7 +197,15 @@
 	               !(ctx->timing && ctx->timing_filter.empty()) &&
 	               !ctx->step_hook;
 	ss.verdict.pending = false;
-	ss.ahead_map_ok = false; ss.ahead_ready = false;
+	const uint64_t launched0 = ss.launched, failed0 = ss.failed;
+	const bool pipelined_call = ss.pipelined;
+	const bool known_arrays = same_bodies_arrays(*a->bodies, ss.lay_bodies) && same_collider_arrays(*a->colliders, ss.lay_colliders) && a->contacts->data == ss.lay_contacts.data && a->contacts->tags == ss.lay_contacts.tags &&
+	                 a->contacts->sleeping_pairs == ss.lay_contacts.sleeping_pairs && a->active_bodies->indices == ss.lay_active && a->contact_cache->data == ss.cache_data && a->contact_cache->tags == ss.cache_tags && a->contact_cache->features == ss.cache_features;
+	if (!ss.pipelined || !known_arrays || steps == 0u) nh_carry_drop(ctx);
+	ss.carry_adopt = ss.carry_out == 1u && !ss.no_carry && ss.ahead_map_ok && !ctx->halo_split.armed;
+	if (ss.carry_adopt) { ss.ahead_ready = true; ss.pair_ready = true; }
+	else { carry_void(ss); ss.ahead_map_ok = false; ss.ahead_ready = false; }
+	ss.in_step = true;
 	int result = NH_OK;
 	uint32_t i = 0;
 	while (i < steps || ss.verdict.pending) {
@@ -222,7 +248,11 @@
 		    (rc = nh_advance(ctx, a->active_bodies, a->bodies, a->time_step))) { result = rc; break; }
 		++i;
 	}
-	ss.pipelined = false; ss.more_steps = false; ss.ahead_ready = false; ss.ahead_map_ok = false; ss.steps_left = 0u; ss.substep = 0u; ss.own_current = false;
+	ss.in_step = false; ss.carry_adopt = false;
+	if (result || ss.verdict.pending) nh_carry_drop(ctx);
+	if (ss.carry_out != 1u) { carry_void(ss); ss.ahead_map_ok = false; }
+	if (!result && pipelined_call && ss.launched - launched0 == steps && ss.failed == failed0) { if (ss.calls_steady < 0xffffu) ss.calls_steady++; } else ss.calls_steady = 0u;
+	ss.pipelined = false; ss.more_steps = false; ss.ahead_ready = false; ss.steps_left = 0u; ss.substep = 0u; ss.own_current = false;
 	if (result && ss.verdict.pending) { if (ss.verdict.event) hipEventSynchronize(ss.ev_ring[ss.verdict.slot]); else hipStreamSynchronize(ctx->stream); ss.verdict.pending = false; }
 	return result;
 }
diff --git a/nudge_amd/engine.py b/nudge_amd/engine.py
--- a/nudge_amd/engine.py
+++ b/nudge_amd/engine.py
@@ -20,7 +20,7 @@
 NH_VIEW_CONTACTS, NH_VIEW_CACHE, NH_VIEW_ACTIVE, NH_VIEW_ALL = 1, 2, 4, 7
 OPTION_NAMES = ("no_still", "no_kept_pairs", "no_incremental", "no_sort_reuse", "sort_radix", "bucket_tile", "bucket_target",
                 "colour_check_seeds", "no_resident", "no_blocks", "blk_check", "blk_min", "blk_target", "blk_rows_global",
-                "blk_global_colours", "blk_profile", "no_asleep", "no_blk_chain", "no_local_still", "no_xform_ahead", "sync_exports_views", "no_pair_ahead", "no_sleeper_skip", "halo_overlap", "no_early_counts", "no_sleeper_ahead", "no_listed_lookup")
+                "blk_global_colours", "blk_profile", "no_asleep", "no_blk_chain", "no_local_still", "no_xform_ahead", "sync_exports_views", "no_pair_ahead", "no_sleeper_skip", "halo_overlap", "no_early_counts", "no_sleeper_ahead", "no_listed_lookup", "no_carry")
 
 EXPORTS = [
     "nh_create", "nh_destroy", "nh_set_flags", "nh_synchronize", "nh_read_counts", "nh_export_views", "nh_set_cache_count",
@@ -77,7 +77,7 @@
     _fields_ = [(n, C.c_uint32) for n in ("colliders", "pairs", "contacts", "sleeping_pairs", "active_bodies", "cache", "culled",
                                           "large_colliders", "general_contacts", "levels", "error", "has_other_bodies", "unleveled", "raw_pairs", "broadphase_rebuilds", "sort_reuses", "broadphase_inserts",
                                           "still_steps", "still_replays", "still_diff_key", "still_diff_count", "still_diff_feature", "still_diff_escape",
-                                          "blk_blocks", "blk_bodies", "blk_ghosts", "asleep_steps", "ahead_steps", "fused_steps", "pair_steps", "pair_diag_roles", "pair_diag_record", "pair_diag_scale", "pair_diag_owned")]
+                                          "blk_blocks", "blk_bodies", "blk_ghosts", "asleep_steps", "ahead_steps", "fused_steps", "pair_steps", "pair_diag_roles", "pair_diag_record", "pair_diag_scale", "pair_diag_owned", "carry_steps", "carry_failed")]
 
     def as_dict(self):
         return {n: int(getattr(self, n)) for n, _ in self._fields_}
```

Result: no change. 3912 (-0.6%).
